# uci-rendering/psdr-cuda

Measured on AMD Instinct MI355X. Metric: Mpath-samples/s renderC+renderD, cbox 512x512 spp=64; grad rel-L2 vs ref, higher is better.
Workload: dtype f32; 1 GPU; cbox 512x512 spp=64/GPU PathTracer(max_depth=3): renderC + configure + renderD + enoki.forward w.r.t. diffuse albedo, through the psdr_cuda surface; triangles=12, global_spp=64, world_size=1, device=AMD Radeon Graphics, local_rank=0

## Files before the change

__graft_entry__.py:

```python
import os
import subprocess
import sys

ROOT = os.path.dirname(os.path.abspath(__file__))
PKG = os.path.join(ROOT, "psdr-cuda_amd")
for p in (PKG, os.path.join(ROOT, "oracle"), os.path.join(ROOT, "tests")):
    if p not in sys.path:
        sys.path.insert(0, p)

HIPCC_FLAGS = ["--offload-arch=gfx950", "-O3", "-std=c++17", "-fPIC", "-munsafe-fp-atomics",
               "-fno-hip-fp32-correctly-rounded-divide-sqrt", "-fgpu-flush-denormals-to-zero", "-fno-slp-vectorize",
               "-freciprocal-math", "-fapprox-func"]
VARIANTS = (0, 1, 2, 3, 4, 6, 8, 10)


def _stale(target, sources):
    return (not os.path.exists(target)) or any(os.path.getmtime(s) > os.path.getmtime(target) for s in sources)


def build():
    csrc = os.path.join(PKG, "csrc")
    srcs = [os.path.join(csrc, f) for f in os.listdir(csrc)] + [os.path.join(ROOT, "include", "psdr_hip.h")]
    lib = os.path.join(PKG, "lib", "libpsdr_hip.so")
    os.makedirs(os.path.dirname(lib), exist_ok=True)
    defect_job = None
    if _stale(lib, srcs):
        obj_dir = os.path.join(PKG, "lib", "obj")
        os.makedirs(obj_dir, exist_ok=True)
        jobs, objs, unit_cmds = [], [], {}
        for v in VARIANTS:
            o = os.path.join(obj_dir, "variant%d.o" % v)
            objs.append(o)
            unit_cmds[o] = ["hipcc"] + HIPCC_FLAGS + ["-DPSDR_VARIANT_FLAGS=%d" % v, "-c", os.path.join(csrc, "psdr_variant.hip"), "-o", o]
            jobs.append(subprocess.Popen(unit_cmds[o]))
            o = os.path.join(obj_dir, "path_sedge%d.o" % v)
            objs.append(o)
            unit_cmds[o] = ["hipcc"] + HIPCC_FLAGS + ["-DPSDR_VARIANT_FLAGS=%d" % v, "-c", os.path.join(csrc, "psdr_path_sedge.hip"), "-o", o]
            jobs.append(subprocess.Popen(unit_cmds[o]))
        o = os.path.join(obj_dir, "logd_lean.o")
        objs.append(o)
        unit_cmds[o] = ["hipcc"] + HIPCC_FLAGS + ["-c", os.path.join(csrc, "psdr_logd_lean.hip"), "-o", o]
        jobs.append(subprocess.Popen(unit_cmds[o]))
        o = os.path.join(obj_dir, "host.o")
        objs.append(o)
        unit_cmds[o] = ["hipcc"] + HIPCC_FLAGS + ["-c", os.path.join(csrc, "psdr_hip.hip"), "-o", o]
        jobs.append(subprocess.Popen(unit_cmds[o]))
        o = os.path.join(obj_dir, "tables.o")
        objs.append(o)
        unit_cmds[o] = ["hipcc"] + HIPCC_FLAGS + ["-c", os.path.join(csrc, "psdr_tables.hip"), "-o", o]
        jobs.append(subprocess.Popen(unit_cmds[o]))
        defect_job = _start_defect_object(csrc, obj_dir)
        if any(j.wait() != 0 for j in jobs):
            raise RuntimeError("hipcc failed")
        sys.path.insert(0, os.path.join(ROOT, "tools"))
        import check_spill_exec
        fallbacks = (["-mllvm", "-amdgpu-opt-exec-mask-pre-ra=0"], ["-mllvm", "-amdgpu-spill-sgpr-to-vgpr=0"])
        from concurrent.futures import ThreadPoolExecutor
        with ThreadPoolExecutor(max_workers=8) as pool:
            first = dict(zip(unit_cmds, pool.map(lambda o_: check_spill_exec.check_library(o_, verbose=True, min_code_objects=1), list(unit_cmds))))
        for o, cmd in list(unit_cmds.items()):
            hits = first[o]
            for extra in fallbacks:
                if not hits:
                    break
                print("build(): %s trips the spill guard -- rebuilding it with %s" % (os.path.basename(o), " ".join(extra)))
                subprocess.check_call(cmd[:1] + cmd[1:-4] + extra + cmd[-4:])
                hits = check_spill_exec.check_library(o, verbose=True, min_code_objects=1)
            if hits:
                raise RuntimeError("%s: %d kernel(s) spill in front of an exec restore with every fallback (tools/check_spill_exec.py)" % (os.path.basename(o), len(hits)))
        subprocess.check_call(["hipcc", "--offload-arch=gfx950", "-shared", "-fPIC"] + objs + ["-o", lib])
        if len(check_spill_exec.code_objects(lib)) < len(objs):
            raise RuntimeError("the linked library holds fewer gfx code objects than translation units: the spill guard cannot see all of it")
    subprocess.check_call(["make", "-C", os.path.join(ROOT, "oracle"), "-s"])
    hc_dir = os.path.join(ROOT, "tests", "hostcheck")
    hc = os.path.join(hc_dir, "libhostcheck.so")
    if _stale(hc, srcs + [os.path.join(hc_dir, "hostcheck.cpp")]):
        subprocess.check_call(["hipcc", "--offload-arch=gfx950", "-O2", "-std=c++17", "-fPIC", "-shared", "-pthread",
                               os.path.join(hc_dir, "hostcheck.cpp"), "-o", hc])
    hp = os.path.join(hc_dir, "libhostcheck_path_sedge.so")
    if _stale(hp, srcs + [os.path.join(hc_dir, "hostcheck_path_sedge.cpp")]):
        subprocess.check_call(["hipcc", "--offload-arch=gfx950", "-O2", "-std=c++17", "-fPIC", "-shared", "-pthread",
                               os.path.join(hc_dir, "hostcheck_path_sedge.cpp"), "-o", hp])
    po_dir = os.path.join(ROOT, "tests", "poison")
    po = os.path.join(po_dir, "libpoison.so")
    if _stale(po, [os.path.join(po_dir, "poison.hip")]):
        subprocess.check_call(["hipcc", "--offload-arch=gfx950", "-O1", "-fPIC", "-shared", os.path.join(po_dir, "poison.hip"), "-o", po])
    try:
        build_defect_lib(defect_job)
    except Exception as e:
        print("build(): tests/poison/libpsdr_hip_defect.so not built (%s) -- only tests/test_rough_rev_order_gpu.py uses it" % e)
    import psdr_cuda
    from psdr_cuda import _abi
    _abi.load_hip()
    import oracle
    oracle.load_oracle()


def _defect_object_cmd(csrc, obj_dir):
    return ["hipcc"] + HIPCC_FLAGS + ["-DPSDR_VARIANT_FLAGS=10", "-DPSDR_SINK_REG_PRIV_ROUGH=1", "-DPSDR_DPP_ALWAYS=1", "-c",
                                      os.path.join(csrc, "psdr_variant.hip"), "-o", os.path.join(obj_dir, "variant10_defect.o")]


def _start_defect_object(csrc, obj_dir):
    try:
        return subprocess.Popen(_defect_object_cmd(csrc, obj_dir), stdout=subprocess.DEVNULL, stderr=subprocess.DEVNULL)
    except Exception:
        return None


def build_defect_lib(object_job=None):
    csrc = os.path.join(PKG, "csrc")
    srcs = [os.path.join(csrc, f) for f in os.listdir(csrc)] + [os.path.join(ROOT, "include", "psdr_hip.h")]
    obj_dir = os.path.join(PKG, "lib", "obj")
    defect_lib = os.path.join(ROOT, "tests", "poison", "libpsdr_hip_defect.so")
    objs = [os.path.join(obj_dir, "%s%d.o" % (unit, v)) for v in VARIANTS for unit in ("variant", "path_sedge")] + [os.path.join(obj_dir, "logd_lean.o"), os.path.join(obj_dir, "host.o"), os.path.join(obj_dir, "tables.o")]
    if not all(os.path.exists(o) for o in objs):
        return None
    if object_job is not None and object_job.wait() != 0:
        object_job = None
    if _stale(defect_lib, srcs + objs):
        defect_obj = os.path.join(obj_dir, "variant10_defect.o")
        if object_job is None:
            subprocess.check_call(_defect_object_cmd(csrc, obj_dir))
        subprocess.check_call(["hipcc", "--offload-arch=gfx950", "-shared", "-fPIC"] + [defect_obj if o.endswith("variant10.o") else o for o in objs] + ["-o", defect_lib])
    return defect_lib


def smoke():
    import numpy as np
    import torch
    assert torch.cuda.is_available(), "smoke() needs a GPU"
    torch.cuda.set_device(0)
    import oracle
    from helpers import GpuScene, load_scene, rel_l2, tangents_wrt
    from psdr_cuda import _abi
    sc, P = load_scene("cbox", res=32, spp=8, sppe=4, sppse=4, translate=(0, (1.0, 0.0, 0.0)))
    tb = sc.tables(0)
    g = GpuScene(tb)
    o = _abi.make_opts(integrator=_abi.INTEGRATOR_PATH, max_depth=3, spp=8)
    img = g.render_c(o)
    ref = oracle.render(tb, o)
    assert np.isfinite(img).all() and rel_l2(img, ref) < 1e-4, rel_l2(img, ref)
    o = _abi.make_opts(spp=8, sppe=4, sppse=4)
    tan = tangents_wrt(tb, P)
    img, dimg = g.render_d_fwd(o, [tan])
    rimg, rd = oracle.render(tb, o, mode=1, tangents=tan)
    assert rel_l2(img, rimg) < 1e-4 and rel_l2(dimg[0], rd) < 1e-3, (rel_l2(img, rimg), rel_l2(dimg[0], rd))
    import psdr_cuda
    from psdr_cuda.fixtures import scene_path
    s2 = psdr_cuda.Scene()
    s2.load_file(scene_path("cbox"), False)
    s2.opts.width = s2.opts.height = 32
    s2.opts.spp, s2.opts.sppe, s2.opts.sppse, s2.opts.log_level = 4, 0, 0, 0
    s2.configure()
    out = psdr_cuda.DirectIntegrator(1, 1).renderC(s2).numpy()
    assert out.shape == (32 * 32, 3) and np.isfinite(out).all() and out.mean() > 0.05
    print("smoke OK: renderC rel-L2 vs oracle %.2e" % rel_l2(img, rimg))


if __name__ == "__main__":
    build()
    if len(sys.argv) > 1 and sys.argv[1] == "smoke":
        smoke()
    if len(sys.argv) > 1 and sys.argv[1] == "defect":
        print(build_defect_lib())
```

include/psdr_hip.h:

```cpp
#ifndef PSDR_HIP_H
#define PSDR_HIP_H

#include <stdint.h>

#ifdef __cplusplus
extern "C" {
#endif

#define PSDR_TRI_STRIDE   24
#define PSDR_TRIUV_STRIDE  8
#define PSDR_SEDGE_STRIDE 16
#define PSDR_PEDGE_STRIDE  8
#define PSDR_BSDF_STRIDE  16
#define PSDR_EMITTER_F_STRIDE 8
#define PSDR_EMITTER_I_STRIDE 4
#define PSDR_CAM_WORDS    64
#define PSDR_ENV_WORDS    32

#define PSDR_TRI_FACE_NORMALS 0x40000000

#define PSDR_BSDF_DIFFUSE        0
#define PSDR_BSDF_ROUGHCONDUCTOR 1
#define PSDR_SLOT_REFLECTANCE 0
#define PSDR_SLOT_ALPHA_U     1
// ... 102 lines not shown
    float *g_prim_edge;
    float *g_env_f;
} psdr_grads;

typedef struct psdr_scene_s *psdr_scene_t;

const char *psdr_last_error(void);
const char *psdr_version(void);
int psdr_abi_struct_sizes(int32_t out[4]);

int psdr_scene_create(psdr_scene_t *out);
int psdr_scene_destroy(psdr_scene_t h);
int psdr_scene_set_option(psdr_scene_t h, const char *name, double value);

int psdr_scene_set_tables(psdr_scene_t h, const psdr_scene_desc *desc);

int psdr_bvh_build(psdr_scene_t h, void *stream);
int psdr_bvh_stats(psdr_scene_t h, int32_t out[4]);
int psdr_scene_info(psdr_scene_t h, int32_t out[8]);

int psdr_trace(psdr_scene_t h, int32_t m,
               const float *ox, const float *oy, const float *oz,
               const float *dx, const float *dy, const float *dz,
               const float *tmax,
               int32_t *out_shape, int32_t *out_tri, float *out_u, float *out_v,
               void *stream);

int psdr_render_c(psdr_scene_t h, const psdr_render_opts *opts,
                  float *out_img, void *stream);

int psdr_render_d_fwd(psdr_scene_t h, const psdr_render_opts *opts,
                      int32_t K, const psdr_tangents *tangents,
                      float *out_img, float *out_dimg, void *stream);

int psdr_render_d_rev(psdr_scene_t h, const psdr_render_opts *opts,
                      const float *adj_img, float *out_img,
                      const psdr_grads *grads, void *stream);

int psdr_guide_build(psdr_scene_t h, const psdr_render_opts *opts,
                     const int32_t reso[4], int32_t nrounds,
                     float *out_mass, void *stream);

int psdr_cube_sample_reuse(int32_t ndim, const int32_t *reso, const float *cmf, const float *pmf, float sum,
                           int32_t n, int32_t m, float *samples, float *out_pdf, void *stream);
int psdr_sample_boundary_segment_direct(const psdr_scene_desc *desc, int32_t m, const float *sample3,
                                        const uint8_t *active, float *out_p0, float *out_edge_dir,
                                        float *out_edge2, float *out_p2, float *out_n, float *out_pdf,
                                        uint8_t *out_valid, int32_t *out_edge, float *out_s1, void *stream);

int psdr_geo_world_vertices_fwd(int32_t V, const float *v_raw, const int32_t *vmesh, const float *mats, float *v_world, void *stream);
int psdr_geo_world_vertices_rev(int32_t V, const float *v_raw, const int32_t *vmesh, const float *mats, const float *v_world, const float *a_world, float *a_raw,
                                void *stream);
int psdr_geo_world_vertices_jvp(int32_t V, const float *v_raw, const int32_t *vmesh, const float *mats, const float *v_world, const float *t_raw, const float *t_mats,
                                float *t_world, void *stream);
int psdr_geo_tri_rows_fwd(int32_t V, int32_t T, const float *v, const int32_t *faces, float *vsum, float *rows, int32_t row_stride, void *stream);
int psdr_geo_tri_rows_rev(int32_t V, int32_t T, const float *v, const int32_t *faces, const float *vsum, const float *a_rows, int32_t row_stride,
                          float *a_vsum , float *a_v, void *stream);
int psdr_geo_tri_rows_jvp(int32_t V, int32_t T, const float *v, const int32_t *faces, const float *vsum, const float *t_v, int32_t row_stride,
                          float *t_vsum , float *t_rows, void *stream);
int psdr_geo_sec_edges_fwd(int32_t E, const int32_t *edges, const float *v, const float *rows, int32_t row_stride, float *info, uint8_t *keep, void *stream);
int psdr_geo_sec_edges_rev(int32_t E, const int32_t *edges, const float *a_info, float *a_v, float *a_rows, int32_t row_stride, void *stream);
int psdr_geo_sec_edges_jvp(int32_t E, const int32_t *edges, const float *t_v, const float *t_rows, int32_t row_stride, float *t_info, void *stream);
int psdr_geo_prim_edges_fwd(int32_t E, const int32_t *edges, const uint8_t *face_normals, const float *v, const float *rows, int32_t row_stride,
                            const float *cam22, float *rows8, float *z4, uint8_t *keep, void *stream);
int psdr_geo_prim_edges_rev(int32_t E, const int32_t *edges, const float *v, const float *cam22, const float *a_rows8, float *a_v, float *a_w2s ,
                            void *stream);
int psdr_geo_prim_edges_jvp(int32_t E, const int32_t *edges, const float *v, const float *cam22, const float *t_v, const float *t_w2s , float *t_rows8,
                            void *stream);

int psdr_geo_compact_edges_fwd(int32_t E, const float *rows, int32_t S, const uint8_t *keep, int32_t w0, int32_t wn, const void *aux, int32_t aux_stride, int32_t A,
                               void *scratch, float *rows_out, void *aux_out, int32_t *pos, float *pmf, float *cmf, float *header, void *stream);
int psdr_geo_compact_edges_rev(int32_t E, int32_t S, const int32_t *pos, const float *a_rows_out, float *a_rows, void *stream);
int psdr_geo_compact_edges_jvp(int32_t E, int32_t S, const int32_t *pos, const float *t_rows, float *t_rows_out, void *stream);
int psdr_geo_emitter_tables(int32_t M, const float *rows, int32_t row_stride, const int32_t *face_offset, const int32_t *mesh_emitter, int32_t Ne, const int32_t *emitter_i,
                            const float *radiance, const float *env_weight, float *mesh_area, float *emitter_f, float *emitter_pmf, float *emitter_cmf, float *face_pmf,
                            float *face_cmf, void *stream);

int psdr_scene_rev_layout(psdr_scene_t h, int32_t out[16]);

int psdr_scene_seed_info(psdr_scene_t h, int64_t out[4]);

int psdr_scene_logd_info(psdr_scene_t h, int64_t out[4]);

int psdr_get_counters(psdr_scene_t h, uint64_t out[4]);

#ifdef __cplusplus
}
#endif
#endif
```

psdr-cuda_amd/csrc/psdr_device.h:

```cpp
#pragma once
#include "psdr_math.h"
#include "../../include/psdr_hip.h"

namespace psdr {

struct __attribute__((aligned(16))) BvhNode {
    float lo0[3], hi0[3];
    float lo1[3], hi1[3];
    int32_t c0, c1;
    int32_t pad[2];
};
static_assert(sizeof(BvhNode) == 64, "BvhNode must be 64 bytes");

struct __attribute__((aligned(16))) Bvh4Node {
    float org[3];
    uint32_t exps;
    uint32_t qlo[3], qhi[3];
    int32_t child[4];
    uint32_t pad[2];
};
static_assert(sizeof(Bvh4Node) == 64, "Bvh4Node must be 64 bytes");
constexpr int32_t kNoChild = 0x7ffffffe;

constexpr int kBvhStack = 40;
// ... 328 lines not shown
    if (sc.nodes4 != nullptr) walk_tree4<IGN>(sc, st, o, d, inv, root4, best, ig0, ig1);
    else walk_tree<IGN>(sc, st, o, d, inv, root2, best, ig0, ig1);
#else
    (void) root4; walk_tree<IGN>(sc, st, o, d, inv, root2, best, ig0, ig1);
#endif
}

#ifndef PSDR_PE_PAIR
#define PSDR_PE_PAIR 1
#endif
PSDR_HD void walk_tree_pair(const SceneView &sc, TraversalStack &st, const Vec3f &o, const Vec3f &dA, const Vec3f &invA, const Vec3f &dB, const Vec3f &invB, int32_t root,
                            Hit &bestA, Hit &bestB) {
    int sp = 0;
    int32_t cur = root;
    constexpr int32_t kDone = 0x7fffffff;
    while (cur != kDone) {
        while (cur >= 0 && cur != kDone) {
            BvhNode n;
#if defined(__HIP_DEVICE_COMPILE__)
            if (cur < sc.n_lnodes) n = *reinterpret_cast<const BvhNode *>(psdr_dyn_lds + sc.off_lnodes + cur * kLdsNodeStride);
            else
#endif
                n = sc.nodes[cur];
            float a0, a1, b0, b1;
            const bool hA0 = slab(n.lo0, n.hi0, o, invA, bestA.t, a0), hA1 = slab(n.lo1, n.hi1, o, invA, bestA.t, a1);
            const bool hB0 = slab(n.lo0, n.hi0, o, invB, bestB.t, b0), hB1 = slab(n.lo1, n.hi1, o, invB, bestB.t, b1);
            const bool h0 = hA0 || hB0, h1 = hA1 || hB1;
            if (h0 && h1) {
                const float t0 = fminf(hA0 ? a0 : INFINITY, hB0 ? b0 : INFINITY), t1 = fminf(hA1 ? a1 : INFINITY, hB1 ? b1 : INFINITY);
                const bool first0 = t0 <= t1;
                st.put(sp++, first0 ? n.c1 : n.c0);
                cur = first0 ? n.c0 : n.c1;
            } else if (h0 || h1) {
                cur = h0 ? n.c0 : n.c1;
            } else {
                cur = sp > 0 ? st.get(--sp) : kDone;
            }
        }
        if (cur == kDone) break;
        {
            const int enc = ~cur, first = enc >> 3, cnt = (enc & 7) + 1;
#if defined(__HIP_DEVICE_COMPILE__)
            if (first + cnt <= sc.n_lbtris) {
                const float4 *lt = reinterpret_cast<const float4 *>(psdr_dyn_lds + sc.off_lbtris) + first * 3;
                for (int i = 0; i < cnt; ++i) {
                    const float4 ta = lt[i * 3], tb = lt[i * 3 + 1], tc = lt[i * 3 + 2];
                    leaf_triangle_test<false>(ta, tb, tc, o, dA, bestA);
                    leaf_triangle_test<false>(ta, tb, tc, o, dB, bestB);
                }
            } else
#endif
            {
                const float4 *bt = sc.btris + (size_t) first * 3;
                for (int i = 0; i < cnt; ++i) {
                    const float4 ta = bt[i * 3], tb = bt[i * 3 + 1], tc = bt[i * 3 + 2];
                    leaf_triangle_test<false>(ta, tb, tc, o, dA, bestA);
                    leaf_triangle_test<false>(ta, tb, tc, o, dB, bestB);
                }
            }
            cur = sp > 0 ? st.get(--sp) : kDone;
        }
    }
}

PSDR_HD bool blas_box(const SceneView &sc, int k, const Vec3f &o, const Vec3f &inv, float tmax, float &t_entry) {
    const float lo[3] = {sc.blas_lo[k].x, sc.blas_lo[k].y, sc.blas_lo[k].z}, hi[3] = {sc.blas_hi[k].x, sc.blas_hi[k].y, sc.blas_hi[k].z};
    return slab(lo, hi, o, inv, tmax, t_entry);
}

PSDR_HD uint32_t wave_or_hd(uint32_t x) {
#if defined(__HIP_DEVICE_COMPILE__)
    unsigned long long todo = __ballot(1);
    uint32_t u = 0u;
    while (todo != 0ull) {
        const uint32_t f = (uint32_t) __builtin_amdgcn_readlane((int) x, __ffsll((long long) todo) - 1);
        u |= f;
        todo &= ~__ballot(x == f);
    }
    return u;
#else
    return x;
#endif
}
template <bool IGN = false, int FOREST = -1, bool MASKED = false>
PSDR_HD Hit closest_hit(const SceneView &sc, TraversalStack &st, const Vec3f &o, const Vec3f &d, float tmax, int ig0 = -1, int ig1 = -1, int pre_slot = 0, uint32_t rows = 0xffffffffu) {
    Hit best; best.tri = -1; best.u = best.v = -1.f;
    best.t = (tmax > 0.f && tmax < INFINITY) ? __int_as_float_hd(__float_as_int_hd(tmax) + 1) : tmax;
    const Vec3f inv{1.f / d.x, 1.f / d.y, 1.f / d.z};
    const bool forest = FOREST < 0 ? sc.n_blas > 0 : FOREST == 1;
    if (FOREST == 3 || FOREST == 2 || sc.n_tiny > 0 || forest) {
        int best_i = kNoPrim;
#if defined(__HIP_DEVICE_COMPILE__)
        typedef __attribute__((address_space(4))) const float4 kernarg_float4;
        const kernarg_float4 *prim_rows = (kernarg_float4 *) ((__attribute__((address_space(4))) const char *) __builtin_amdgcn_kernarg_segment_ptr() + offsetof(SceneView, tiny));
#else
        const float4 *prim_rows = sc.tiny;
#endif
        const int aa_cnt = sc.aa_cnt;
        if (aa_cnt != 0) {
            float4 ra[kAaSlots]; float hb[kAaSlots]; int pk[kAaSlots], id2[kAaSlots];
#pragma unroll
            for (int i = 0; i < kAaSlots; ++i) {
                ra[i] = prim_rows[i * 4];
                if (IGN) { const float4 r = prim_rows[i * 4 + 1]; hb[i] = r.x; pk[i] = __float_as_int_hd(r.y); id2[i] = __float_as_int_hd(r.w); }
                else {
#if defined(__HIP_DEVICE_COMPILE__)
                    const float2 r = *(__attribute__((address_space(4))) const float2 *) &prim_rows[i * 4 + 1];
#else
                    const float2 r{prim_rows[i * 4 + 1].x, prim_rows[i * 4 + 1].y};
#endif
                    hb[i] = r.x; pk[i] = __float_as_int_hd(r.y); id2[i] = 0;
                }
            }
            const int cx = aa_cnt & 255, cy = (aa_cnt >> 8) & 255, cz = aa_cnt >> 16;
#define PSDR_AA(AX, S) do { if (!MASKED || ((rows >> (S)) & 1u) != 0u) aa_prim_test<AX, IGN>(ra[S], hb[S], pk[S], id2[S], o, d, inv, best, best_i, ig0, ig1); } while (0)
            if (cx > 0) { PSDR_AA(0, 0); if (cx > 1) { PSDR_AA(0, 1); if (cx > 2) PSDR_AA(0, 2); } }
            if (cy > 0) { PSDR_AA(1, 3); if (cy > 1) { PSDR_AA(1, 4); if (cy > 2) PSDR_AA(1, 5); } }
            if (cz > 0) { PSDR_AA(2, 6); if (cz > 1) { PSDR_AA(2, 7); if (cz > 2) PSDR_AA(2, 8); } }
#undef PSDR_AA
        }
#pragma unroll PSDR_TINY_UNROLL
        for (int i = aa_cnt != 0 ? kAaSlots : 0; i < sc.n_tiny; ++i)
            if (!MASKED || ((rows >> i) & 1u) != 0u) tiny_prim_test<IGN>(prim_rows[i * 4], prim_rows[i * 4 + 1], prim_rows[i * 4 + 2], prim_rows[i * 4 + 3], i, o, d, best, best_i, ig0, ig1);
        resolve_tiny_hit(sc, best, best_i);
        if (FOREST == 3) {
            const Hit ph = st.pre[pre_slot];
            if (ph.tri >= 0 && ph.t < best.t) best = ph;
            return best;
        }
        if (FOREST == 2 || !forest) return best;
        if (sc.n_blas == 1) {
            float te;
            if (blas_box(sc, 0, o, inv, best.t, te)) walk<IGN>(sc, st, o, d, inv, __float_as_int_hd(sc.blas_lo[0].w), __float_as_int_hd(sc.blas_hi[0].w), best, ig0, ig1);
            return best;
        }
        uint32_t cand = (1u << sc.n_blas) - 1u;
        while (cand) {
            int32_t root = 0, root4 = 0; float near_t = INFINITY; uint32_t pick = 0;
            for (int k = 0; k < sc.n_blas; ++k) {
                if (!((cand >> k) & 1u)) continue;
                float te;
                if (!blas_box(sc, k, o, inv, best.t, te)) cand &= ~(1u << k);
                else if (te < near_t) { near_t = te; root = __float_as_int_hd(sc.blas_lo[k].w); root4 = __float_as_int_hd(sc.blas_hi[k].w); pick = 1u << k; }
            }
            if (!pick) break;
            cand &= ~pick;
            walk<IGN>(sc, st, o, d, inv, root, root4, best, ig0, ig1);
        }
        return best;
    }
    walk<IGN>(sc, st, o, d, inv, sc.root, sc.root4, best, ig0, ig1);
    return best;
}

template <int FLAGS> constexpr bool pair_walk_ok() { return PSDR_PE_PAIR != 0 && tree_mode<FLAGS>() == 1 && PSDR_WIDE_TREE == 0; }
PSDR_HD void closest_hit_pair(const SceneView &sc, TraversalStack &st, const Vec3f &o, const Vec3f &dA, const Vec3f &dB, Hit &hA, Hit &hB) {
#pragma unroll 1
    for (int r = 0; r < 2; ++r) {
        const Hit h = closest_hit<false, 2>(sc, st, o, r ? dB : dA, INFINITY);
        if (r) hB = h; else hA = h;
    }
    const Vec3f invA{1.f / dA.x, 1.f / dA.y, 1.f / dA.z}, invB{1.f / dB.x, 1.f / dB.y, 1.f / dB.z};
    for (int k = 0; k < sc.n_blas; ++k) {
        float te;
        const bool eA = blas_box(sc, k, o, invA, hA.t, te), eB = blas_box(sc, k, o, invB, hB.t, te);
        if (eA || eB) walk_tree_pair(sc, st, o, dA, invA, dB, invB, __float_as_int_hd(sc.blas_lo[k].w), hA, hB);
    }
}

template <class R> struct Loader;
template <> struct Loader<float> {
    template <int KK, int E> static PSDR_HD float f(const float *tab, const TangentView<KK, E> &, const float *const psdr_tangents::*, size_t i) { return tab[i]; }
};
template <int K> struct Loader<Dual<K>> {
    template <int E> static PSDR_HD Dual<K> f(const float *tab, const TangentView<K, E> &tv, const float *const psdr_tangents::*m, size_t i) {
        Dual<K> r; r.v = tab[i];
#pragma unroll
        for (int k = 0; k < K; ++k) { const float *p = tv.t[k].*m; r.d[k] = p ? p[i] : 0.f; }
        return r;
    }
};
template <class R, int FLAGS = kSceneRough> using TV = TangentView<ad_traits<R>::K, FLAGS>;
template <class R, class TVT> PSDR_HD R ldf(const float *tab, const TVT &tv, const float *const psdr_tangents::*m, size_t i) {
    return Loader<R>::f(tab, tv, m, i);
}
template <class R, class TVT> PSDR_HD Vec3<R> ld3(const float *tab, const TVT &tv, const float *const psdr_tangents::*m, size_t i) {
    return {ldf<R>(tab, tv, m, i), ldf<R>(tab, tv, m, i + 1), ldf<R>(tab, tv, m, i + 2)};
}
template <class M> PSDR_HD M to_m(float x) { return M(x); }
template <class M, int K> PSDR_HD M to_m(const Dual<K> &x) { return x; }
template <class M, class G> PSDR_HD Vec3<M> to_m3(const Vec3<G> &a) { return {to_m<M>(a.x), to_m<M>(a.y), to_m<M>(a.z)}; }

template <class R> struct TriRow { Vec3<R> p0, e1, e2, n0, n1, n2, fn; R area; };
template <class TVT> PSDR_HD TriRow<float> load_tri_f(const SceneView &sc, const TVT &, int id) {
    TriRow<float> t;
    float4 r[6];
#if defined(__HIP_DEVICE_COMPILE__)
    if (TVT::tiny || id < sc.n_ltri) {
        const float4 *q = reinterpret_cast<const float4 *>(psdr_dyn_lds + sc.off_ltri) + (size_t) id * 6;
#pragma unroll
        for (int i = 0; i < 6; ++i) r[i] = q[i];
    } else
#endif
    {
        const float4 *q = reinterpret_cast<const float4 *>(sc.d.tri_info) + (size_t) id * 6;
#pragma unroll
// ... 191 lines not shown
}

constexpr float kInvTwoPi = 0.15915494309189533577f;
template <class M, class G, class TVT> PSDR_HD Vec3<M> env_eval_direction(const SceneView &sc, const TVT &tv, const Vec3<G> &w) {
    const float *f = sc.d.env_f;
    constexpr auto m = &psdr_tangents::d_env_f;
    const Vec3<M> wm = to_m3<M>(w);
    auto row = [&](int r) {
        return ldf<M>(f, tv, m, PSDR_ENV_FROM_WORLD + r * 3) * wm.x + ldf<M>(f, tv, m, PSDR_ENV_FROM_WORLD + r * 3 + 1) * wm.y +
               ldf<M>(f, tv, m, PSDR_ENV_FROM_WORLD + r * 3 + 2) * wm.z;
    };
    const M vx = row(0), vy = row(1), vz = row(2);
    M u = atan2_(vx, -vz) * kInvTwoPi, v = safe_acos_(vy) * kInvPi;
    u = u - floorf(val(u)); v = v - floorf(val(v));
    M rgb[3];
    bitmap_eval<M, 3>(sc, tv, sc.d.env_tex, u, v, rgb, false);
    const M scale = ldf<M>(f, tv, m, PSDR_ENV_SCALE);
    return {rgb[0] * scale, rgb[1] * scale, rgb[2] * scale};
}
template <class M, class G, class TVT> PSDR_HD Vec3<M> Le(const SceneView &sc, const TVT &tv, const Its<G> &its, bool active) {
    const int e = active ? emitter_of(sc, tv, its) : -1;
    if (e < 0) return zero3<M>();
    if (TVT::has_env && e == sc.d.env_emitter) return env_eval_direction<M>(sc, tv, -its.sh.to_world(its.wi));
    if (!(val(its.wi.z) > 0.f)) return zero3<M>();
    return radiance<M>(sc, tv, e);
}


template <class R> struct GGX {
    R au, av;
    PSDR_HD R eval(const Vec3<R> &m) const {
        const R r = 1.f / (kPi * au * av * sqr(sqr(m.x / au) + sqr(m.y / av) + sqr(m.z)));
        return val(r) * val(m.z) > 1e-5f ? r : R(0.f);
    }
    PSDR_HD R smith_g1(const Vec3<R> &v, const Vec3<R> &m) const {
        const R xy = sqr(au * v.x) + sqr(av * v.y);
        R r = 2.f / (1.f + sqrt_(1.f + xy / sqr(v.z)));
        if (val(xy) == 0.f) r = R(1.f);
        if (val(dot(v, m)) * val(v.z) <= 0.f) r = R(0.f);
        return r;
    }
    PSDR_HD void visible11(const R &cos_i, float sx, float sy, R &ox, R &oy) const {
        float px, py;
        concentric_disk(sx, sy, px, py);
        const R s = 0.5f * (1.f + cos_i);
        const R y = sqrtf(fmaxf(1.f - px * px, 0.f)) * (1.f - s) + py * s;
        const R z = safe_sqrt(1.f - (px * px + y * y));
        const R sin_i = safe_sqrt(1.f - sqr(cos_i));
        const R nrm = 1.f / (sin_i * y + cos_i * z);
        ox = (cos_i * y - sin_i * z) * nrm; oy = px * nrm;
    }
    PSDR_HD Vec3<R> sample(const Vec3<R> &wi, float sx, float sy) const {
        const Vec3<R> wp = normalize(Vec3<R>(au * wi.x, av * wi.y, wi.z));
        const R st2 = wp.x * wp.x + wp.y * wp.y;
        R sin_phi(0.f), cos_phi(1.f);
        if (!(fabsf(val(st2)) <= 4.f * kEpsilon)) {
            const R inv = 1.f / sqrt_(st2);
            sin_phi = clamp_(wp.y * inv, -1.f, 1.f); cos_phi = clamp_(wp.x * inv, -1.f, 1.f);
        }
        R slx, sly;
        visible11(wp.z, sx, sy, slx, sly);
        const R s0 = (cos_phi * slx - sin_phi * sly) * au, s1 = (sin_phi * slx + cos_phi * sly) * av;
        return normalize(Vec3<R>(-s0, -s1, R(1.f)));
    }
};

template <class R> PSDR_HD R fresnel_conductor(const R &eta, const R &k, const R &cos_i) {
    const R c2 = sqr(cos_i), s2 = 1.f - c2, s4 = sqr(s2);
    const R t1 = sqr(eta) - sqr(k) - s2;
    const R a2pb2 = safe_sqrt(sqr(t1) + 4.f * sqr(k * eta));
    const R a = safe_sqrt(0.5f * (a2pb2 + t1));
    const R T1 = a2pb2 + c2, T2 = 2.f * cos_i * a;
    const R rs = (T1 - T2) / (T1 + T2);
    const R T3 = a2pb2 * c2 + s4, T4 = T2 * s2;
    return 0.5f * (rs + rs * (T3 - T4) / (T3 + T4));
}

template <class M> struct MatCache { M au, av; Vec3<M> eta, k, refl; };
template <class G, class M> struct Bsdf {
    const int32_t *rec;
    const MatCache<M> *mc = nullptr;
    PSDR_HD Bsdf(const SceneView &sc, int id) : rec(sc.d.bsdf_rec + (size_t) (id < 0 ? 0 : id) * PSDR_BSDF_STRIDE) {}
    template <class TVT> PSDR_HD Bsdf(const SceneView &sc, const TVT &, int id) : rec(Tab<TVT::flags>::bsdf_rec(sc, id)) {}
    template <class TVT> PSDR_HD MatCache<M> fetch(const SceneView &sc, const TVT &tv, const Its<G> &its) const {
        MatCache<M> c;
        c.refl = tex3(sc, tv, PSDR_SLOT_REFLECTANCE, its);
        if (is_diffuse(tv)) { c.au = c.av = M(0.f); c.eta = c.k = zero3<M>(); return c; }
        c.au = tex1(sc, tv, PSDR_SLOT_ALPHA_U, its); c.av = tex1(sc, tv, PSDR_SLOT_ALPHA_V, its);
        c.eta = tex3(sc, tv, PSDR_SLOT_ETA, its); c.k = tex3(sc, tv, PSDR_SLOT_K, its);
        return c;
    }
    PSDR_HD int type() const { return rec[0]; }
    template <class TVT> PSDR_HD bool is_diffuse(const TVT &) const { return !TVT::has_rough || rec[0] == PSDR_BSDF_DIFFUSE; }
    PSDR_HD const int32_t *slot(int s) const { return rec + 1 + 3 * s; }
    template <class TVT> PSDR_HD Vec3<M> tex3(const SceneView &sc, const TVT &tv, int s, const Its<G> &its) const {
        if (mc) return s == PSDR_SLOT_ETA ? mc->eta : (s == PSDR_SLOT_K ? mc->k : mc->refl);
        M o[3]; bitmap_eval<M, 3>(sc, tv, slot(s), its.uvx, its.uvy, o); return {o[0], o[1], o[2]};
    }
    template <class TVT> PSDR_HD M tex1(const SceneView &sc, const TVT &tv, int s, const Its<G> &its) const {
        if (mc) return s == PSDR_SLOT_ALPHA_U ? mc->au : mc->av;
        M o[1]; bitmap_eval<M, 1>(sc, tv, slot(s), its.uvx, its.uvy, o); return o[0];
    }
    template <class TVT> PSDR_HD Vec3<M> eval(const SceneView &sc, const TVT &tv, const Its<G> &its, const Vec3<G> &wo, bool active) const {
        if (!(active && val(its.wi.z) > 0.f && val(wo.z) > 0.f)) return zero3<M>();
        if (is_diffuse(tv)) return tex3(sc, tv, PSDR_SLOT_REFLECTANCE, its) * (wo.z * kInvPi);
        const GGX<M> g{tex1(sc, tv, PSDR_SLOT_ALPHA_U, its), tex1(sc, tv, PSDR_SLOT_ALPHA_V, its)};
        const Vec3<M> wi_m = to_m3<M>(its.wi), wo_m = to_m3<M>(wo);
        const Vec3<M> H = normalize(wo_m + wi_m);
        const M D = g.eval(H);
        if (val(D) == 0.f) return zero3<M>();
        const M res = D * (g.smith_g1(wi_m, H) * g.smith_g1(wo_m, H)) / (4.f * wi_m.z);
        const Vec3<M> eta = tex3(sc, tv, PSDR_SLOT_ETA, its), k = tex3(sc, tv, PSDR_SLOT_K, its);
        const M c = dot(wi_m, H);
        const Vec3<M> F{fresnel_conductor(eta.x, k.x, c), fresnel_conductor(eta.y, k.y, c), fresnel_conductor(eta.z, k.z, c)};
        return F * res * tex3(sc, tv, PSDR_SLOT_REFLECTANCE, its);
    }
    template <class TVT> PSDR_HD M pdf(const SceneView &sc, const TVT &tv, const Its<G> &its, const Vec3<G> &wo, bool active) const {
        if (is_diffuse(tv)) {
            const float ci = val(its.wi.z), co = val(wo.z);
            return M((active && ci > 0.f && co > 0.f) ? kInvPi * co : 0.f);
        }
        const Vec3<M> wi_m = to_m3<M>(its.wi);
        const Vec3<M> m = normalize(to_m3<M>(wo) + wi_m);
        const GGX<M> g{tex1(sc, tv, PSDR_SLOT_ALPHA_U, its), tex1(sc, tv, PSDR_SLOT_ALPHA_V, its)};
        return g.eval(m) * g.smith_g1(wi_m, m) / (4.f * wi_m.z);
    }
    template <class TVT> PSDR_HD bool sample(const SceneView &sc, const TVT &tv, const Its<G> &its, const float s[3], bool active, Vec3f &wo,
                                             M &pdf_) const {
        if (is_diffuse(tv)) {
            wo = cosine_hemisphere(s[1], s[2]);
            pdf_ = M(kInvPi * wo.z);
            return active && val(its.wi.z) > 0.f;
        }
        const GGX<M> g{tex1(sc, tv, PSDR_SLOT_ALPHA_U, its), tex1(sc, tv, PSDR_SLOT_ALPHA_V, its)};
        const Vec3<M> wi_m = to_m3<M>(its.wi);
        const Vec3<M> m = g.sample(wi_m, s[0], s[1]);
        const Vec3<M> wo_m = m * (2.f * dot(wi_m, m)) - wi_m;
        const Vec3<M> h = normalize(wo_m + wi_m);
        pdf_ = g.eval(h) * g.smith_g1(wi_m, h) / (4.f * wi_m.z);
        wo = val(wo_m);
        return active && val(its.wi.z) > 0.f && val(pdf_) != 0.f && wo.z > 0.f;
    }
};

template <class R> struct PosSample { Vec3<R> p, n; R J; float pdf; bool valid; int tri; };

template <int NDIM>
PSDR_HD float cube_sample_reuse(const float *__restrict__ cmf, const float *__restrict__ pmf, float sum, int n, int r0, int r1, int r2, float s[NDIM]) {
    static_assert(NDIM == 2 || NDIM == 3, "cube_sample_reuse: 2 or 3 dimensions");
    float p;
    const int idx = sample_reuse(cmf, pmf, sum, n, s[NDIM - 1], p);
    if constexpr (NDIM == 2) {
        const int c0 = idx / r1, c1 = idx - c0 * r1;
        s[0] = (s[0] + (float) c0) * (1.f / (float) r0);
        s[1] = (s[1] + (float) c1) * (1.f / (float) r1);
    } else {
        const int c0 = idx / (r1 * r2), rem = idx - c0 * r1 * r2, c1 = rem / r2, c2 = rem - c1 * r2;
        s[0] = (s[0] + (float) c0) * (1.f / (float) r0);
        s[1] = (s[1] + (float) c1) * (1.f / (float) r1);
        s[2] = (s[2] + (float) c2) * (1.f / (float) r2);
    }
    return p * (float) n;
}

PSDR_HD float env_cells_sample_reuse(const SceneView &sc, float &u0, float &u1) {
    const int r0 = sc.d.env_reso[0], r1 = sc.d.env_reso[1];
// ... 696 lines not shown
```

psdr-cuda_amd/csrc/psdr_hip.hip:

```cpp
#define PSDR_WIDE_TREE 2
#include "psdr_host.h"
#include "psdr_bvh_build.h"

#include <cstdlib>
#include <cstring>
#include <rocprim/rocprim.hpp>

namespace {
__global__ __launch_bounds__(kBlock) void k_trace(LaunchCtx cx, int m, const float *__restrict__ ox, const float *__restrict__ oy,
                                                  const float *__restrict__ oz, const float *__restrict__ dx,
                                                  const float *__restrict__ dy, const float *__restrict__ dz,
                                                  const float *__restrict__ tmax, int32_t *__restrict__ out_shape,
                                                  int32_t *__restrict__ out_tri, float *__restrict__ out_u, float *__restrict__ out_v) {
    TraversalStack st; setup_lds(cx, st);
    const SceneView &sc = cx.sc;
    for (int i = blockIdx.x * kBlock + threadIdx.x; i < m; i += gridDim.x * kBlock) {
        const Hit h = closest_hit<false, -1>(sc, st, Vec3f{ox[i], oy[i], oz[i]}, Vec3f{dx[i], dy[i], dz[i]}, tmax[i]);
        out_tri[i] = h.tri;
        out_shape[i] = h.tri >= 0 ? (sc.d.tri_mesh[h.tri] & ~PSDR_TRI_FACE_NORMALS) : -1;
        out_u[i] = h.u; out_v[i] = h.v;
    }
}


// ... 393 lines not shown
        if (hipMallocAsync(&nb, need, s) != hipSuccess) { (void) hipGetLastError(); nb = nullptr; }
    }
    if (*buf) HIP_TRY(hipFreeAsync(*buf, s));
    *buf = nullptr; *have = 0;
    if (nb == nullptr) {
        if (hipMallocAsync(&nb, need, s) != hipSuccess) {
            (void) hipGetLastError();
            return fail(std::string("psdr: could not allocate ") + std::to_string(need >> 20) + " MB of device memory for the " + what);
        }
    }
    *buf = nb; *have = need;
    return 0;
}

int launch_blocks(const psdr_scene_s *h, long long n, int per_cu) {
    const int forced = h->opt.blocks_per_cu;
    const long long need = (n + kBlock - 1) / kBlock;
    const long long cap = (long long) h->num_cus * (forced ? forced : per_cu);
    return (int) std::max(1LL, std::min(need, cap));
}

constexpr int kLdsBudget = 40 * 1024;
static bool tiny_only(const psdr_scene_s *h) { return h->n_tiny > 0 && h->n_blas == 0; }
static int emitter_faces(const psdr_scene_s *h) {
    int n = 0;
    for (int e = 0; e < h->desc.num_emitters && (size_t) (e + 1) * PSDR_EMITTER_I_STRIDE <= h->emitter_i.size(); ++e)
        n = std::max(n, h->emitter_i[(size_t) e * PSDR_EMITTER_I_STRIDE + 3] + h->emitter_i[(size_t) e * PSDR_EMITTER_I_STRIDE + 2]);
    return n;
}
constexpr int kLdsTexels = 256, kLdsTexelTangents = 3;
static bool small_tables_fit(const psdr_scene_s *h) {
    const psdr_scene_desc &d = h->desc;
    return d.env_emitter < 0 && d.num_meshes <= 64 && d.num_bsdfs <= 32 && d.num_emitters >= 0 && d.num_emitters <= 8 &&
           (d.num_emitters == 0 || (d.face_cmf && d.face_pmf)) && emitter_faces(h) <= 64;
}
static bool tiny_tables_ok(const psdr_scene_s *h) {
    return h->opt.tiny_variants != 0 && tiny_only(h) && small_tables_fit(h);
}
static bool forest_tables(const psdr_scene_s *h) { return PSDR_FOREST_LDS_TABLES && h->n_blas > 0; }
static bool use_wide_tree(const psdr_scene_s *h, bool forest) {
    if (h->opt.wide == 0) return false;
    return forest && h->has_rough && h->desc.env_emitter < 0;
}

static int stack_entries_of(const psdr_scene_s *h) { return tiny_only(h) ? 0 : (h->wide ? h->stack_need4 + 1 : std::min(kBvhStack, h->bvh_depth + 2)); }
static int staged_nodes_of(const psdr_scene_s *h) { return h->wide ? h->num_nodes4 : h->num_nodes; }
int plan_lds(const psdr_scene_s *h, LaunchCtx &cx, int reserved) {
    const int forced = h->opt.lds_budget;
    const bool lean = !h->has_rough && h->desc.env_emitter < 0;
    const int budget = forced ? forced : (lean ? 28 * 1024 : kLdsBudget);
    const int stack_bytes = stack_entries_of(h) * kBlock * 4;
    int room = std::max(0, budget - reserved - stack_bytes);
    if (tiny_only(h)) room = std::max(room, staged_nodes_of(h) * kLdsNodeStride + h->num_btris * 48 + h->desc.num_tris * 96);
    SceneView &sc = cx.sc;
    int off = 0;
    sc.n_lnodes = std::min(staged_nodes_of(h), room / kLdsNodeStride); sc.off_lnodes = off; off += sc.n_lnodes * kLdsNodeStride; room -= sc.n_lnodes * kLdsNodeStride;
    sc.n_lbtris = (sc.n_lnodes == staged_nodes_of(h)) ? std::min(h->num_btris, room / 48) : 0;
    sc.off_lbtris = off; off += sc.n_lbtris * 48; room -= sc.n_lbtris * 48;
    sc.n_ltri = (sc.n_lbtris == h->num_btris) ? std::min(h->desc.num_tris, room / 96) : 0;
    sc.off_ltri = off; off += sc.n_ltri * 96;
    sc.off_lprim = off; off += h->n_tiny * kTinyHitWords * 4;
    sc.lt_trimesh = sc.lt_meshbsdf = sc.lt_meshemitter = sc.lt_bsdf = sc.lt_emf = sc.lt_emi = sc.lt_fcmf = sc.lt_fpmf = sc.lt_uv = sc.lt_tex = sc.lt_ecmf = sc.lt_epmf = -1;
    sc.lt_nfaces = 0; sc.lt_occ = -1; sc.occ = nullptr;
    const bool all_tables = tiny_tables_ok(h);
    if (all_tables || forest_tables(h)) {
        auto take = [&](int words) { const int o = off; off += (words * 4 + 15) / 16 * 16; return o; };
        const psdr_scene_desc &d = h->desc;
        sc.lt_nfaces = emitter_faces(h);
        if (all_tables) sc.lt_trimesh = take(d.num_tris);
        sc.lt_meshbsdf = take(d.num_meshes); sc.lt_meshemitter = take(d.num_meshes);
        sc.lt_bsdf = take(std::max(d.num_bsdfs, 1) * PSDR_BSDF_STRIDE);
        sc.lt_emf = take(d.num_emitters * PSDR_EMITTER_F_STRIDE); sc.lt_emi = take(d.num_emitters * PSDR_EMITTER_I_STRIDE);
        sc.lt_fcmf = take(sc.lt_nfaces); sc.lt_fpmf = take(sc.lt_nfaces);
        if (d.num_emitters > 1 && d.emitter_cmf && d.emitter_pmf) { sc.lt_ecmf = take(d.num_emitters); sc.lt_epmf = take(d.num_emitters); }
        if (all_tables && d.tri_uv) sc.lt_uv = take(d.num_tris * PSDR_TRIUV_STRIDE);
        if (d.num_texels > 0 && d.num_texels <= kLdsTexels) sc.lt_tex = take(d.num_texels * (1 + kLdsTexelTangents));
        if (all_tables && h->have_occ && h->d_occ != nullptr) { sc.occ = h->d_occ; sc.lt_occ = take(d.num_tris * d.num_tris); }
    }
    sc.lt_end = off;
    cx.off_stack = off;
    return off + stack_bytes;
}
int lds_bytes(const LaunchCtx &cx, const psdr_scene_s *h) { return cx.off_stack + stack_entries_of(h) * kBlock * 4; }

void fill_top(const psdr_scene_s *h, SceneView &sc) {
    sc.n_tiny = h->n_tiny; sc.aa_cnt = h->n_tiny > 0 ? h->aa_cnt : 0;
    sc.emit_rows = (h->n_tiny > 0 && h->opt.emitter_pretest != 0) ? h->emit_rows : 0u;
    std::memcpy(sc.tiny, h->tiny, sizeof(h->tiny));
    std::memcpy(sc.tiny_meta, h->tiny_meta, sizeof(h->tiny_meta));
    sc.n_blas = h->n_blas;
    std::memcpy(sc.blas_lo, h->blas_lo, sizeof(h->blas_lo));
    std::memcpy(sc.blas_hi, h->blas_hi, sizeof(h->blas_hi));
    for (int k = 0; k < h->n_blas; ++k) std::memcpy(&sc.blas_hi[k].w, &h->blas_root4[k], 4);
    sc.nodes4 = h->wide ? h->d_nodes4 : nullptr; sc.root4 = h->root4;
}

int make_ctx(psdr_scene_s *h, const psdr_render_opts *o, int sampler, LaunchCtx &cx) {
    if (!h->have_tables) return fail("Scene not loaded yet!");
    if (!h->have_bvh) return fail("Input scene must be configured!");
    if (o->integrator != PSDR_INTEGRATOR_FIELD && h->desc.num_emitters <= 0) return fail("No Emitter!");
    if (o->integrator == PSDR_INTEGRATOR_DIRECT && !(o->bsdf_samples >= 0 && o->light_samples >= 0 && o->bsdf_samples + o->light_samples > 0))
        return fail("DirectIntegrator: bsdf_samples + light_samples must be positive");
    cx.sc.d = h->desc; cx.sc.nodes = h->d_nodes; cx.sc.btris = h->d_btris; cx.sc.root = h->root;
    fill_top(h, cx.sc);
    plan_lds(h, cx);
    cx.sc.literal_forms = (o->flags & PSDR_FLAG_LITERAL_FORMS) ? 1 : 0;
    cx.lp = LiParams{o->integrator, o->bsdf_samples, o->light_samples, o->max_depth, o->hide_emitters, o->field};
    cx.jump = make_rng_jump(o->rng_offset[sampler]);
    return 0;
}

int check_path_sedges(const psdr_render_opts *o) {
    if (o->integrator == PSDR_INTEGRATOR_PATH && (o->flags & PSDR_FLAG_PATH_SEDGES) != 0 && o->sppse > 0 && o->max_depth > PSDR_PATH_SEDGES_MAX_DEPTH)
        return fail("PSDR_FLAG_PATH_SEDGES: PathTracer max_depth > 8 is not supported for the secondary-edge term");
    return 0;
}
int check_counts(const psdr_scene_s *h, const psdr_render_opts *o) {
    const long long WH = (long long) h->desc.width * h->desc.height;
    if (WH <= 0) return fail("Invalid film resolution");
    if (WH * std::max(o->spp, 1) > 0x7fffffffLL) return fail("Too many samples (width*height*spp > INT_MAX)");
    if (o->spp_begin < 0 || o->spp_end > o->spp || o->spp_begin > o->spp_end) return fail("Invalid spp shard range");
    if (o->sppe_begin < 0 || o->sppe_end > o->sppe || o->sppe_begin > o->sppe_end) return fail("Invalid sppe shard range");
    if (o->sppse_begin < 0 || o->sppse_end > o->sppse || o->sppse_begin > o->sppse_end) return fail("Invalid sppse shard range");
    return 0;
}

bool open_scene(const psdr_scene_s *h) { return !(h->n_blas > 0 || (h->n_tiny > 0 && h->n_blas == 0)); }
bool use_wavefront(const psdr_scene_s *h, const psdr_render_opts *o) {
    if (o->integrator != PSDR_INTEGRATOR_PATH || o->max_depth > 250) return false;
    if (h->desc.num_tris >= (1 << 29)) return false;
    if (o->flags & PSDR_FLAG_FUSED) return false;
    if (o->flags & PSDR_FLAG_WAVEFRONT) return true;
    if (o->max_depth < 2) return false;
    if (open_scene(h)) return true;
    const long long n = (long long) h->desc.width * h->desc.height * (o->spp_end - o->spp_begin);
    if (traced_wavefront(h)) return n >= (1ll << 16);
    return h->n_blas > 0 && h->wf_binned && n >= (1ll << 25);
}

SinkLayout make_sink_layout(const psdr_scene_s *h, const psdr_grads *g) {
    SinkLayout L{};
    int off = 0;
    L.cam_off = off; off += 16;
    if (g->g_env_f && h->desc.env_emitter >= 0) { L.env_off = off; L.env_n = PSDR_ENV_WORDS; off += PSDR_ENV_WORDS; }
    const int nt = h->desc.num_texels, nr = h->desc.num_emitters * 3;
    if (g->g_texels && nt > 0 && nt <= 2048) { L.tex_off = off; L.tex_n = nt; off += nt; }
    if (g->g_emitter_rad && nr > 0 && nr <= 256) { L.rad_off = off; L.rad_n = nr; off += nr; }
    if (g->g_tri_info && h->hot_rows > 0) {
        const int rows = std::min(h->hot_rows, (kSinkCacheWords - off) / PSDR_TRI_STRIDE);
        if (rows > 0) { L.hot_off = off; L.hot_rows = rows; L.hot_map = h->d_hot_map; L.hot_tris = h->d_hot_tris; off += rows * PSDR_TRI_STRIDE; }
    }
    L.total = off;
    L.stride = off | 1;
    L.rep = 1;
    const int max_rep = h->opt.sink_rep;
    while (L.rep * 2 <= max_rep && L.rep * 2 * L.stride <= kSinkCacheWords) L.rep *= 2;
    const bool priv_on = h->opt.sink_private != 0;
    L.priv_tri[0] = L.priv_tri[1] = -1; L.priv_slot[0] = L.priv_slot[1] = 0; L.priv_emitter = -1;
    if (priv_on && L.hot_rows > 0 && h->desc.num_emitters > 0 && h->desc.env_emitter != 0) {
        const int32_t *ei = h->emitter_i.data();
        const int n = std::min(std::min(ei[2], 2), L.hot_rows);
        for (int r = 0; r < n; ++r) { L.priv_tri[r] = ei[1] + r; L.priv_slot[r] = h->hot_identity ? ei[1] + r : r; }
        L.priv_rows = n;
        if (n > 0) { L.priv_off = (L.rep * L.stride + 3) / 4 * 4; if (L.rad_n) L.priv_emitter = 0; }
    }
    return L;
// ... 272 lines not shown
    if (tiny_tables_ok(h)) fl |= kSceneTiny;
    switch (fl) {
        case 0: return variant_ops_0();
        case 1: return variant_ops_1();
        case 2: return variant_ops_2();
        case 3: return variant_ops_3();
        case 4: return variant_ops_4();
        case 8: return variant_ops_8();
        case 10: return variant_ops_10();
        default: return variant_ops_6();
    }
}
const PathSedgeOps *path_sedge_of(const psdr_scene_s *h) {
    int fl = (h->desc.env_emitter >= 0 ? kSceneEnv : 0) | (h->has_rough ? kSceneRough : 0) | (h->n_blas > 0 ? kSceneForest : 0);
    if (tiny_tables_ok(h)) fl |= kSceneTiny;
    switch (fl) {
        case 0: return path_sedge_ops_0();
        case 1: return path_sedge_ops_1();
        case 2: return path_sedge_ops_2();
        case 3: return path_sedge_ops_3();
        case 4: return path_sedge_ops_4();
        case 8: return path_sedge_ops_8();
        case 10: return path_sedge_ops_10();
        default: return path_sedge_ops_6();
    }
}
}
using namespace psdr_host;

extern "C" {

const char *psdr_last_error(void) { return g_err.c_str(); }
const char *psdr_version(void) { return "psdr-hip 0.1 gfx950"; }
int psdr_abi_struct_sizes(int32_t out[4]) {
    out[0] = (int32_t) sizeof(psdr_scene_desc); out[1] = (int32_t) sizeof(psdr_render_opts);
    out[2] = (int32_t) sizeof(psdr_tangents); out[3] = (int32_t) sizeof(psdr_grads);
    return 0;
}

int psdr_scene_create(psdr_scene_t *out) {
    if (!out) return fail("psdr_scene_create: null output");
    psdr_scene_s *h = new psdr_scene_s();
    hipError_t e = hipMalloc(&h->d_counters, sizeof(unsigned long long) * kRayCounters * kRayCounterStride);
    if (e != hipSuccess) { delete h; return fail(std::string("hipMalloc: ") + hipGetErrorString(e)); }
    int dev = 0; hipDeviceProp_t prop;
    if (hipGetDevice(&dev) == hipSuccess && hipGetDeviceProperties(&prop, dev) == hipSuccess) {
        h->num_cus = prop.multiProcessorCount;
        h->lds_limit = (int) std::min<size_t>(prop.sharedMemPerBlock, 160 * 1024);
    }
    *out = h;
    return 0;
}

int psdr_scene_set_option(psdr_scene_t h, const char *name, double value) {
    if (!h || !name) return fail("psdr_scene_set_option: null argument");
    const std::string n(name);
    const int iv = (int) value;
    if (n == "bvh_refit") h->refit_enabled = iv != 0;
    else if (n == "forest_min_inline") { h->forest_min_inline = iv; h->have_bvh = false; }
    else if (n == "scratch_plain") g_scratch_plain = iv;
    else if (n == "own_pixels") h->opt.own_pixels = iv;
    else if (n == "emitter_pretest") h->opt.emitter_pretest = iv;
    else if (n == "occ_rows") { h->opt.occ_rows = iv; h->have_bvh = false; }
    else if (n == "aa_prims") { h->aa_enabled = iv != 0; h->have_bvh = false; }
    else if (n == "tiny_scene") h->tiny_enabled = iv != 0;
    else if (n == "two_level") h->two_level_enabled = iv != 0;
    else if (n == "wf_binned") h->wf_binned = iv != 0;
    else if (n == "wf_traced") h->traced_enabled = iv != 0;
    else if (n == "bvh_build") h->bvh_device_mode = iv;
    else if (n == "sort_edges") h->sort_edges = iv != 0;
    else if (n == "blocks_per_cu") h->opt.blocks_per_cu = iv;
    else if (n == "camera_blocks") h->opt.camera_blocks = iv;
    else if (n == "tiny_variants") h->opt.tiny_variants = iv;
    else if (n == "wide") h->opt.wide = iv;
    else if (n == "lds_budget") h->opt.lds_budget = iv;
    else if (n == "sink_rep") h->opt.sink_rep = std::max(1, std::min(16, iv));
    else if (n == "sink_private") h->opt.sink_private = iv;
    else if (n == "rev_split") h->opt.rev_split = iv;
    else if (n == "tangent_live") h->opt.tangent_live = iv;
    else if (n == "wf_geo") h->opt.wf_geo = iv;
    else if (n == "logd") h->opt.logd = iv;
    else if (n == "seed_cache") h->opt.seed_cache = iv;
    else if (n == "logd_park") h->opt.logd_park = iv;
    else if (n == "seed_cache_log2") h->opt.seed_cache_log2 = std::max(0, std::min(40, iv));
    else if (n == "keep_records") h->opt.keep_records = iv;
    else if (n == "rev_sorted") h->opt.rev_sorted = iv;
    else if (n == "sedge_split") h->opt.sedge_split = iv;
    else if (n == "pt_sedge") h->opt.pt_sedge = iv & 3;
    else if (n == "pt_sedge_walk") h->opt.pt_sedge_walk = iv;
    else if (n == "probe") h->opt.probe = iv;
    else if (n == "trace_wg2") h->opt.trace_wg2 = iv;
    else if (n == "chunk_log2") h->opt.chunk_log2 = std::max(0, std::min(30, iv));
    else if (n == "bvh_maxleaf") h->opt.bvh_maxleaf = std::max(1, std::min(8, iv));
    else if (n == "bvh_tcost") h->opt.bvh_tcost = (float) value;
    else return fail("psdr_scene_set_option: unknown option '" + n + "'");
    h->kept.valid = false;
    if (n == "tiny_scene" || n == "two_level" || n == "bvh_build" || n == "wide" || n == "bvh_maxleaf" || n == "bvh_tcost" || n == "tiny_variants") h->have_bvh = false;
    return 0;
}

int psdr_scene_destroy(psdr_scene_t h) {
    if (!h) return 0;
    if (h->d_nodes) (void) hipFree(h->d_nodes);
    if (h->d_btris) (void) hipFree(h->d_btris);
    if (h->d_counters) (void) hipFree(h->d_counters);
    if (h->d_refit_area) (void) hipFree(h->d_refit_area);
    if (h->d_sort) (void) hipFree(h->d_sort);
    if (h->d_ws) (void) hipFree(h->d_ws);
    if (h->d_live) (void) hipFree(h->d_live);
    if (h->d_logd_bad) (void) hipFree(h->d_logd_bad);
    if (h->d_seed) (void) hipFree(h->d_seed);
    if (h->seed_event) (void) hipEventDestroy(h->seed_event);
    if (h->d_hot_map) (void) hipFree(h->d_hot_map);
    if (h->d_hot_tris) (void) hipFree(h->d_hot_tris);
    if (h->d_occ) (void) hipFree(h->d_occ);
    if (h->d_top) (void) hipFree(h->d_top);
    if (h->d_inline_ids) (void) hipFree(h->d_inline_ids);
    if (h->d_lbvh) (void) hipFree(h->d_lbvh);
    if (h->d_nodes4) (void) hipFree(h->d_nodes4);
    if (h->d_topo4) (void) hipFree(h->d_topo4);
    if (h->d_rev) (void) hipFree(h->d_rev);
    if (h->d_se_list) (void) hipFree(h->d_se_list);
    if (h->d_rev_deep) (void) hipFree(h->d_rev_deep);
    if (h->d_pe_rep) (void) hipFree(h->d_pe_rep);
    if (h->d_trace_ovf) (void) hipFree(h->d_trace_ovf);
    if (h->d_probe) (void) hipFree(h->d_probe);
    delete h;
    return 0;
}

int psdr_scene_set_tables(psdr_scene_t h, const psdr_scene_desc *desc) {
    if (!h || !desc) return fail("psdr_scene_set_tables: null argument");
    psdr_scene_desc d = *desc;
    if (d.num_tris <= 0 || !d.tri_info || !d.tri_mesh) return fail("Missing meshes!");
    if (!d.cam) return fail("Missing sensor!");
    if (reinterpret_cast<uintptr_t>(d.tri_info) & 15) return fail("psdr_scene_set_tables: tri_info must be 16-byte aligned");
    if (d.width <= 0 || d.height <= 0) return fail("Invalid film resolution");
    if (d.num_meshes <= 0 || !d.mesh_bsdf || !d.mesh_emitter) return fail("psdr_scene_set_tables: mesh_bsdf / mesh_emitter missing");
    if (d.num_bsdfs > 0 && (!d.bsdf_rec || !d.texels)) return fail("psdr_scene_set_tables: bsdf_rec / texels missing");
    if (d.num_emitters > 0 && (!d.emitter_f || !d.emitter_i)) return fail("psdr_scene_set_tables: emitter tables missing");
    if (d.num_emitters > 1 && (!d.emitter_cmf || !d.emitter_pmf)) return fail("psdr_scene_set_tables: emitter distribution missing");
    if (d.num_sec_edges > 0 && (!d.sec_edge || !d.sec_cmf || !d.sec_pmf)) return fail("psdr_scene_set_tables: secondary-edge tables missing");
    if (d.num_prim_edges > 0 && (!d.prim_edge || !d.prim_cmf || !d.prim_pmf)) return fail("psdr_scene_set_tables: primary-edge tables missing");
    if (d.num_prim_edges <= 0) d.prim_edge_z = nullptr;
    if (d.num_guide_cells > 0 && (!d.guide_cmf || !d.guide_pmf)) return fail("psdr_scene_set_tables: guiding tables missing");
    if (!d.env_f) d.env_emitter = -1;
    if (d.env_emitter >= 0) {
        if (d.env_emitter >= d.num_emitters || !d.env_cmf || !d.env_pmf || d.env_reso[0] <= 0 || d.env_reso[1] <= 0 || d.env_tex[1] < 2 ||
            d.env_tex[2] < 2)
            return fail("psdr_scene_set_tables: inconsistent environment-map record");
    }
    if (h->have_tables && (d.tri_info != h->desc.tri_info || d.num_tris != h->desc.num_tris)) h->have_bvh = false;
    if (h->have_tables && (d.emitter_i != h->desc.emitter_i || d.num_emitters != h->desc.num_emitters)) h->have_bvh = false;
    if (!h->have_tables || std::memcmp(&h->desc, &d, sizeof(d)) != 0) { ++h->tables_gen; h->kept.valid = false; }
    h->desc = d;
    h->has_rough = d.material_mask == 0 || (d.material_mask & (1u << PSDR_BSDF_ROUGHCONDUCTOR)) != 0;
    h->have_tables = true;
    return 0;
}

static hipError_t copy_on_stream(void *dst, const void *src, size_t bytes, hipMemcpyKind kind, hipStream_t s) {
    if (hipError_t e = hipMemcpyAsync(dst, src, bytes, kind, s)) return e;
    return hipStreamSynchronize(s);
}
static void update_emit_rows(psdr_scene_s *h) {
    std::vector<char> is_em((size_t) std::max(h->desc.num_tris, 0), 0);
// ... 291 lines not shown
    if (n <= 0 || n > 0x7fffffffLL) return fail("psdr_guide_build: invalid resolution");
    HIP_TRY(hipMemsetAsync(out_mass, 0, sizeof(float) * cells, s));
    return variant_of(h)->guide(h, cx, reso, nrounds, n, out_mass, s);
}

int psdr_cube_sample_reuse(int32_t ndim, const int32_t *reso, const float *cmf, const float *pmf, float sum, int32_t n, int32_t m, float *samples,
                           float *out_pdf, void *stream) {
    if (!reso || !cmf || !pmf || !samples || !out_pdf) return fail("psdr_cube_sample_reuse: null argument");
    if (ndim != 2 && ndim != 3) return fail("psdr_cube_sample_reuse: ndim must be 2 or 3");
    long long cells = 1;
    for (int d = 0; d < ndim; ++d) {
        if (reso[d] <= 0) return fail("psdr_cube_sample_reuse: invalid resolution");
        cells *= reso[d];
    }
    if (cells != (long long) n) return fail("psdr_cube_sample_reuse: n must be the product of the resolution");
    if (m < 0) return fail("psdr_cube_sample_reuse: negative sample count");
    if (m == 0) return 0;
    const dim3 grid((unsigned) ((m + kBlock - 1) / kBlock));
    hipStream_t s = (hipStream_t) stream;
    if (ndim == 2)
        hipLaunchKernelGGL(k_cube_sample_reuse<2>, grid, dim3(kBlock), 0, s, m, cmf, pmf, sum, n, reso[0], reso[1], 1, samples, out_pdf);
    else
        hipLaunchKernelGGL(k_cube_sample_reuse<3>, grid, dim3(kBlock), 0, s, m, cmf, pmf, sum, n, reso[0], reso[1], reso[2], samples, out_pdf);
    HIP_TRY(hipGetLastError());
    return 0;
}

int psdr_sample_boundary_segment_direct(const psdr_scene_desc *desc, int32_t m, const float *sample3, const uint8_t *active, float *out_p0,
                                        float *out_edge_dir, float *out_edge2, float *out_p2, float *out_n, float *out_pdf, uint8_t *out_valid,
                                        int32_t *out_edge, float *out_s1, void *stream) {
    if (!desc || !sample3 || !out_p0 || !out_edge_dir || !out_edge2 || !out_p2 || !out_n || !out_pdf || !out_valid || !out_edge || !out_s1)
        return fail("psdr_sample_boundary_segment_direct: null argument");
    const psdr_scene_desc &d = *desc;
    if (d.num_sec_edges <= 0 || !d.sec_edge || !d.sec_cmf || !d.sec_pmf) return fail("Scene has no secondary edges");
    if (d.num_emitters <= 0 || !d.emitter_f || !d.emitter_i) return fail("No Emitter!");
    if (d.num_emitters > 1 && (!d.emitter_cmf || !d.emitter_pmf)) return fail("psdr_sample_boundary_segment_direct: emitter distribution missing");
    const bool env = d.env_f != nullptr && d.env_emitter >= 0;
    if (env && (d.env_emitter >= d.num_emitters || !d.env_cmf || !d.env_pmf || d.env_reso[0] <= 0 || d.env_reso[1] <= 0))
        return fail("psdr_sample_boundary_segment_direct: inconsistent environment-map record");
    if (d.num_emitters > (env ? 1 : 0) && (d.num_tris <= 0 || !d.tri_info || !d.face_cmf || !d.face_pmf))
        return fail("psdr_sample_boundary_segment_direct: area-light tables missing");
    if (m < 0) return fail("psdr_sample_boundary_segment_direct: negative sample count");
    if (m == 0) return 0;
    SceneView sc{};
    sc.d = d;
    if (!env) sc.d.env_emitter = -1;
    const dim3 grid((unsigned) ((m + kBlock - 1) / kBlock));
    hipStream_t s = (hipStream_t) stream;
    if (env)
        hipLaunchKernelGGL(k_boundary_segment_direct<kSceneEnv>, grid, dim3(kBlock), 0, s, sc, m, sample3, active, out_p0, out_edge_dir, out_edge2, out_p2, out_n,
                           out_pdf, out_valid, out_edge, out_s1);
    else
        hipLaunchKernelGGL(k_boundary_segment_direct<0>, grid, dim3(kBlock), 0, s, sc, m, sample3, active, out_p0, out_edge_dir, out_edge2, out_p2, out_n,
                           out_pdf, out_valid, out_edge, out_s1);
    HIP_TRY(hipGetLastError());
    return 0;
}

int psdr_bvh_stats(psdr_scene_t h, int32_t out[4]) {
    if (!h || !out) return fail("psdr_bvh_stats: null argument");
    out[0] = h->num_builds; out[1] = h->num_refits; out[2] = h->num_nodes; out[3] = h->bvh_depth;
    return 0;
}

int psdr_scene_info(psdr_scene_t h, int32_t out[8]) {
    if (!h || !out) return fail("psdr_scene_info: null argument");
    const int n_slab = (h->aa_cnt & 255) + ((h->aa_cnt >> 8) & 255) + (h->aa_cnt >> 16);
    out[0] = h->n_tiny - (h->aa_cnt != 0 ? kAaSlots - n_slab : 0); out[1] = h->n_blas; out[2] = h->n_inline; out[3] = h->num_btris; out[4] = h->lbvh ? 1 : 0;
    out[5] = n_slab; out[6] = h->have_occ ? 1 : 0; out[7] = h->have_occ ? h->occ_max_rows : 0;
    return 0;
}

int psdr_scene_rev_layout(psdr_scene_t h, int32_t out[16]) {
    if (!h || !out) return fail("psdr_scene_rev_layout: null argument");
    std::copy(std::begin(h->rev_layout), std::end(h->rev_layout), out);
    return 0;
}

int psdr_scene_logd_info(psdr_scene_t h, int64_t out[4]) {
    if (!h || !out) return fail("psdr_scene_logd_info: null argument");
    out[0] = h->logd_launches; out[1] = h->logd_lean_launches; out[2] = h->logd_lean_seeded; out[3] = (int64_t) h->logd_lean_lds + h->logd_lean_park;
    return 0;
}
int psdr_scene_seed_info(psdr_scene_t h, int64_t out[4]) {
    if (!h || !out) return fail("psdr_scene_seed_info: null argument");
    out[0] = h->seed_valid ? h->seed_key[0] * h->seed_key[3] : 0; out[1] = (int64_t) (h->seed_cap * sizeof(ulonglong2)); out[2] = h->seed_fills; out[3] = h->seed_launches;
    return 0;
}

int psdr_get_counters(psdr_scene_t h, uint64_t out[4]) {
    if (!h || !out) return fail("psdr_get_counters: null argument");
    unsigned long long all[kRayCounters * kRayCounterStride], c[1] = {0};
    HIP_TRY(hipMemcpyAsync(all, h->d_counters, sizeof(all), hipMemcpyDeviceToHost, h->last_stream));
    HIP_TRY(hipStreamSynchronize(h->last_stream));
    for (int i = 0; i < kRayCounters; ++i) c[0] += all[i * kRayCounterStride];
#ifdef PSDR_STAGE_CLOCKS
    {
        unsigned long long ph[12] = {0};
        for (int i = 0; i < kRayCounters; ++i) for (int k = 0; k < 12; ++k) ph[k] += all[i * kRayCounterStride + 1 + k];
        std::fprintf(stderr, "stage clocks:");
        for (int k = 0; k < 12; ++k) std::fprintf(stderr, " %llu", ph[k]);
        std::fprintf(stderr, "\n");
    }
#endif
    out[0] = c[0]; out[1] = h->slots[0]; out[2] = h->slots[1]; out[3] = h->slots[2];
    return 0;
}

}
```

psdr-cuda_amd/csrc/psdr_host.h:

```cpp
#pragma once
#include "psdr_device.h"
#include "psdr_reverse.h"

#include <algorithm>
#include <type_traits>
#include <cmath>
#include <cstdio>
#include <cstdlib>
#include <cstring>
#include <string>
#include <vector>

using namespace psdr;

struct LaunchCtx {
    SceneView sc;
    LiParams lp;
    RngJump jump;
    int32_t off_stack;
    int32_t off_pathrec;
    int32_t off_sink;
    int32_t off_park;
};

static_assert(offsetof(LaunchCtx, sc) == 0, "closest_hit reads SceneView::tiny through the kernel-argument segment pointer: LaunchCtx (SceneView first) must be the first kernel argument");

__device__ __forceinline__ void setup_lds(const LaunchCtx &cx, TraversalStack &st) {
#if defined(__HIP_DEVICE_COMPILE__)
    const SceneView &sc = cx.sc;
    float4 *dst = reinterpret_cast<float4 *>(psdr_dyn_lds);
    const float4 *src = sc.nodes4 != nullptr ? reinterpret_cast<const float4 *>(sc.nodes4) : reinterpret_cast<const float4 *>(sc.nodes);
    for (int i = threadIdx.x; i < sc.n_lnodes * 4; i += kBlock) dst[sc.off_lnodes / 16 + (i >> 2) * (kLdsNodeStride / 16) + (i & 3)] = src[i];
    for (int i = threadIdx.x; i < sc.n_lbtris * 3; i += kBlock) dst[sc.off_lbtris / 16 + i] = sc.btris[i];
    src = reinterpret_cast<const float4 *>(sc.d.tri_info);
    for (int i = threadIdx.x; i < sc.n_ltri * 6; i += kBlock) dst[sc.off_ltri / 16 + i] = src[i];
    {
        float *m = reinterpret_cast<float *>(psdr_dyn_lds + sc.off_lprim);
#pragma unroll 1
        for (int i = 0; i < sc.n_tiny; ++i) {
            int32_t tri; float k[6];
            const int w = threadIdx.x & 7;
            const float4 Sm = sc.tiny[i * 4 + 2];
            const float S[4] = {Sm.x, Sm.y, Sm.z, Sm.w};
            tiny_hit_row(sc.tiny_meta + i * 4, (threadIdx.x >> 3) & 1, tri, k, (sc.aa_cnt != 0 && i < kAaSlots) ? S : nullptr);
            const float val = w == 0 ? __int_as_float(tri) : (w == 1 ? k[0] : w == 2 ? k[1] : w == 3 ? k[2] : w == 4 ? k[3] : w == 5 ? k[4] : w == 6 ? k[5] : 0.f);
            if (threadIdx.x < kTinyHitWords) m[i * kTinyHitWords + threadIdx.x] = val;
        }
    }
    if (sc.lt_meshbsdf >= 0) {
        auto stage = [&](int off, const void *table, int words) {
            if (off < 0 || table == nullptr) return;
            const uint32_t *g = static_cast<const uint32_t *>(table);
            uint32_t *l = reinterpret_cast<uint32_t *>(psdr_dyn_lds + off);
#pragma unroll 1
            for (int i = threadIdx.x; i < words; i += kBlock) l[i] = g[i];
        };
        stage(sc.lt_trimesh, sc.d.tri_mesh, sc.d.num_tris);
        stage(sc.lt_meshbsdf, sc.d.mesh_bsdf, sc.d.num_meshes);
        stage(sc.lt_meshemitter, sc.d.mesh_emitter, sc.d.num_meshes);
        stage(sc.lt_bsdf, sc.d.bsdf_rec, sc.d.num_bsdfs * PSDR_BSDF_STRIDE);
        stage(sc.lt_emf, sc.d.emitter_f, sc.d.num_emitters * PSDR_EMITTER_F_STRIDE);
        stage(sc.lt_emi, sc.d.emitter_i, sc.d.num_emitters * PSDR_EMITTER_I_STRIDE);
        stage(sc.lt_ecmf, sc.d.emitter_cmf, sc.d.num_emitters);
        stage(sc.lt_epmf, sc.d.emitter_pmf, sc.d.num_emitters);
        stage(sc.lt_fcmf, sc.d.face_cmf, sc.lt_nfaces);
        stage(sc.lt_fpmf, sc.d.face_pmf, sc.lt_nfaces);
        stage(sc.lt_uv, sc.d.tri_uv, sc.d.num_tris * PSDR_TRIUV_STRIDE);
        stage(sc.lt_tex, sc.d.texels, sc.d.num_texels);
        stage(sc.lt_occ, sc.occ, sc.d.num_tris * sc.d.num_tris);
    }
    st.base = reinterpret_cast<int32_t *>(psdr_dyn_lds + cx.off_stack) + threadIdx.x;
    __syncthreads();
#else
    (void) cx; (void) st;
#endif
}
template <class TVT> __device__ __forceinline__ void setup_lds(const LaunchCtx &cx, TraversalStack &st, const TVT &tv) {
    setup_lds(cx, st);
#if defined(__HIP_DEVICE_COMPILE__)
    if constexpr (Tab<TVT::flags>::lds_small && TVT::k > 0) {
        constexpr int K = TVT::k;
        static_assert(K <= 3, "plan_lds reserves three tangent texel pools");
        if (cx.sc.lt_tex >= 0) {
            float *l = reinterpret_cast<float *>(psdr_dyn_lds + cx.sc.lt_tex);
            const int nt = cx.sc.d.num_texels;
            for (int k = 0; k < K; ++k) {
                const float *g = tv.t[k].d_texels;
                for (int i = threadIdx.x; i < nt; i += kBlock) l[(k + 1) * nt + i] = g ? g[i] : 0.f;
            }
            __syncthreads();
        }
    }
#endif
}

constexpr int kSinkCacheWords = 6144;
struct SinkLayout {
    int tex_off, tex_n;
    int rad_off, rad_n;
    int cam_off;
    int env_off, env_n;
    int hot_off, hot_rows;
    const int32_t *hot_map, *hot_tris;
    int total;
    int rep, stride;
    int priv_off, priv_rows;
    int priv_tri[2], priv_slot[2], priv_emitter;
    int priv_regs;
    int pend_off, pend_rows;
};
constexpr int kPendWords = 10;
constexpr int kPrivRowWords = 13;
constexpr int kPrivWords = 2 * kPrivRowWords + 3;

struct psdr_scene_options {
    int blocks_per_cu = 0;
    int camera_blocks = 0;
    int tiny_variants = 1;
    int wide = -1;
    int lds_budget = 0;
    int sink_rep = 4;
    int sink_private = 1;
    int rev_split = -1;
    int tangent_live = 1;
    int wf_geo = 1;
    int own_pixels = 1;
    int emitter_pretest = 1;
    int occ_rows = 1;
    int logd = 1;
    int keep_records = 1;
    int rev_sorted = 1;
    int pt_sedge = 3;
    int pt_sedge_walk = 1;
    int sedge_split = -1;
    int chunk_log2 = 0;
    int probe = 1;
    int trace_wg2 = -1;
    int seed_cache = 1;
    int seed_cache_log2 = 25;
    int logd_park = 1;
    int bvh_maxleaf = 4;
    float bvh_tcost = 2.0f;
};

struct psdr_scene_s {
    psdr_scene_options opt;
    psdr_scene_desc desc{};
    bool have_tables = false;
    bool has_rough = true;
    int num_cus = 256;
    int lds_limit = 64 * 1024;

    BvhNode *d_nodes = nullptr;
    float4 *d_btris = nullptr;
    size_t cap_nodes = 0, cap_btris = 0;
    int32_t root = 0;
    bool have_bvh = false;
    int bvh_depth = 0, num_nodes = 0, num_btris = 0;
    Bvh4Node *d_nodes4 = nullptr;
    int32_t *d_topo4 = nullptr;
    size_t cap_nodes4 = 0;
    int num_nodes4 = 0, stack_need4 = 0;
    bool wide = false;
    int32_t *d_trace_ovf = nullptr;
    size_t trace_ovf_bytes = 0;
    bool traced_enabled = true;
    int32_t root4 = 0, blas_root4[kMaxBlas] = {};
    bool refit_enabled = true;
    int tree_tris = -1, refits_since_build = 0, num_builds = 0, num_refits = 0;
    std::vector<int> level_start;
    float bvh_pad = 0.f, built_area = 0.f;
    float *d_refit_area = nullptr;

    int bvh_device_mode = -1;
    bool lbvh = false;
    int lbvh_leaves = 0;
    void *d_lbvh = nullptr;
    size_t lbvh_bytes = 0;

    bool tiny_enabled = true, aa_enabled = true;
    int n_tiny = 0, aa_cnt = 0;
    float4 tiny[kTinyRows * 4] = {};
    int32_t tiny_meta[kTinyRows * 4] = {};
    bool two_level_enabled = true, refit_ok = true, wf_binned = true;
    int n_blas = 0, n_inline = 0;
    float4 blas_lo[kMaxBlas] = {}, blas_hi[kMaxBlas] = {};
    float4 *d_top = nullptr;
    int32_t *d_inline_ids = nullptr;

    unsigned long long *d_counters = nullptr;
    hipStream_t last_stream = nullptr;
    hipStream_t refit_stream = nullptr;
    uint64_t slots[3] = {0, 0, 0};
    int last_path_depth = 0;
    int32_t rev_layout[16] = {};

    std::vector<int32_t> emitter_i;
    int32_t *d_hot_map = nullptr, *d_hot_tris = nullptr;
    uint32_t *d_occ = nullptr; size_t occ_cap = 0; bool have_occ = false; int occ_max_rows = 0;
    int hot_rows = 0;
    bool hot_identity = false;
    size_t hot_cap = 0;

    bool sort_edges = true;
    void *d_sort = nullptr;
    size_t sort_bytes = 0;

    void *d_pe_rep = nullptr;
    size_t pe_rep_bytes = 0;

    void *d_rev_deep = nullptr;
    size_t rev_deep_bytes = 0;

    void *d_se_list = nullptr;
    size_t se_list_bytes = 0;

    void *d_rev = nullptr;
    size_t rev_bytes = 0;
    void *d_logd_bad = nullptr; size_t logd_bad_bytes = 0;
    struct KeptRecords { bool valid = false; psdr_render_opts o{}; uint64_t gen = 0; long long n = 0; int kind = 0; } kept;
    uint64_t tables_gen = 0;

    void *d_seed = nullptr;
    size_t seed_cap = 0;
    long long seed_key[4] = {0, 0, 0, 0};
    bool seed_valid = false;
    hipStream_t seed_stream = nullptr;
    hipEvent_t seed_event = nullptr;
    long long seed_fills = 0, seed_launches = 0;
    long long logd_launches = 0, logd_lean_launches = 0, logd_lean_seeded = 0;
    int logd_lean_lds = 0, logd_lean_park = 0;
    void *d_ws = nullptr;
    size_t ws_bytes = 0;
    void *d_live = nullptr;
    size_t live_bytes = 0;
    void *d_probe = nullptr;
    size_t probe_bytes = 0;
    uint32_t emit_rows = 0;
    int forest_min_inline = 0;
};

constexpr int kRayCounters = 64, kRayCounterStride = 16;
constexpr int kWfSub = 64, kWfCountStride = 32;

namespace psdr_host {
int fail(const std::string &m);
int scratch_reserve(void **buf, size_t *have, size_t need, hipStream_t s, const char *what);
long long fit_chunk(long long chunk, size_t bytes_per_slot, size_t fixed_bytes, size_t have);
inline int workspace_reserve(psdr_scene_s *h, size_t need, hipStream_t s) { return scratch_reserve(&h->d_ws, &h->ws_bytes, need, s, "wavefront workspace (path-state streams + trace requests)"); }
int launch_blocks(const psdr_scene_s *h, long long n, int per_cu = 16);
int plan_lds(const psdr_scene_s *h, LaunchCtx &cx, int reserved = 0);
int lds_bytes(const LaunchCtx &cx, const psdr_scene_s *h);
void fill_top(const psdr_scene_s *h, SceneView &sc);
constexpr int kMaxInlineTris = 2 * kTinyTris;
int make_ctx(psdr_scene_s *h, const psdr_render_opts *o, int sampler, LaunchCtx &cx);
bool use_wavefront(const psdr_scene_s *h, const psdr_render_opts *o);
bool traced_wavefront(const psdr_scene_s *h);
int launch_wf_trace(psdr_scene_s *h, const float4 *req, const int32_t *count, long long sub_cap, float4 *hit, hipStream_t s, bool ign = false);
struct ProbeBuffers { float4 *hit; uint32_t *mask; float4 *req; int32_t *count; long long sub_cap; };
int probe_buffers(psdr_scene_s *h, long long slots, int rays_per_slot, ProbeBuffers &pb, hipStream_t s, int per_cu = 16);
SinkLayout make_sink_layout(const psdr_scene_s *h, const psdr_grads *g);
inline int sink_bytes_base(const SinkLayout &L) { return (L.priv_rows > 0 && !L.priv_regs) ? (L.priv_off + kPrivWords * kBlock) * 4 : (L.rep * L.stride * 4 + 15) / 16 * 16; }
inline int sink_bytes(const SinkLayout &L) { return L.pend_rows > 0 ? (L.pend_off + L.pend_rows * kPendWords * kBlock) * 4 : sink_bytes_base(L); }
inline void sink_reserve_pending(SinkLayout &L, int rows) { L.pend_rows = 0; L.pend_off = (sink_bytes_base(L) / 4 + 3) / 4 * 4; L.pend_rows = rows; }
int check_counts(const psdr_scene_s *h, const psdr_render_opts *o);
int begin_call(psdr_scene_s *h, hipStream_t s);
int primary_edge_order(psdr_scene_s *h, const LaunchCtx &cx, long long i0, long long n, const uint32_t **order, hipStream_t s);
constexpr int kMaxRefits = 64;
constexpr float kRefitAreaGrowth = 1.3f;

struct VariantOps {
    int (*render_c)(psdr_scene_s *h, const psdr_render_opts *o, float *img, hipStream_t s);
    int (*render_fwd)(psdr_scene_s *h, const psdr_render_opts *o, int K, const psdr_tangents *tangents, float *img, float *dimg, hipStream_t s);
    int (*render_rev)(psdr_scene_s *h, const psdr_render_opts *o, const float *adj_img, float *out_img, const psdr_grads *grads, hipStream_t s);
    int (*guide)(psdr_scene_s *h, LaunchCtx &cx, const int32_t reso[4], int nrounds, long long n, float *out_mass, hipStream_t s);
};
struct PathSedgeOps {
    int (*fwd)(psdr_scene_s *h, const psdr_render_opts *o, int K, const psdr_tangents *tangents, float *dimg, hipStream_t s);
    int (*rev)(psdr_scene_s *h, const psdr_render_opts *o, const float *adj_img, const psdr_grads *grads, hipStream_t s);
};
const PathSedgeOps *path_sedge_ops_0();
const PathSedgeOps *path_sedge_ops_1();
const PathSedgeOps *path_sedge_ops_2();
const PathSedgeOps *path_sedge_ops_3();
const PathSedgeOps *path_sedge_ops_4();
const PathSedgeOps *path_sedge_ops_6();
const PathSedgeOps *path_sedge_ops_8();
const PathSedgeOps *path_sedge_ops_10();
int logd_lean_launch_8(psdr_scene_s *h, const psdr_render_opts *o, const LaunchCtx &cx, const psdr::TangentView<1, psdr::kSceneTiny> &tv, float *img, float *dimg, hipStream_t s, bool *ran);
const VariantOps *variant_ops_0();
const VariantOps *variant_ops_1();
const VariantOps *variant_ops_2();
const VariantOps *variant_ops_3();
const VariantOps *variant_ops_4();
const VariantOps *variant_ops_6();
const VariantOps *variant_ops_8();
const VariantOps *variant_ops_10();
}

#define HIP_TRY(expr)                                                                              \
    do { hipError_t e_ = (expr); if (e_ != hipSuccess) return psdr_host::fail(std::string(#expr) + ": " + hipGetErrorString(e_)); } while (0)
```

psdr-cuda_amd/csrc/psdr_kernels.h:

```cpp
#pragma once
#include "psdr_host.h"

namespace {
using namespace psdr_host;

__device__ __forceinline__ float wave_shfl_down(float v, int off) { return __shfl_down(v, off, 64); }

template <int CTRL, int ROW_MASK> __device__ __forceinline__ float dpp_add(float v) {
    return v + __int_as_float(__builtin_amdgcn_update_dpp(0, __float_as_int(v), CTRL, ROW_MASK, 0xf, true));
}
__device__ __forceinline__ float wave_total(float v) {
    v = dpp_add<0x111, 0xf>(v); v = dpp_add<0x112, 0xf>(v); v = dpp_add<0x114, 0xf>(v); v = dpp_add<0x118, 0xf>(v);
    v = dpp_add<0x142, 0xa>(v); v = dpp_add<0x143, 0xc>(v);
    return __int_as_float(__builtin_amdgcn_readlane(__float_as_int(v), 63));
}
#ifndef PSDR_DPP_ALWAYS
#define PSDR_DPP_ALWAYS 0
#endif
template <int N, bool DPP = (N <= 6 || PSDR_DPP_ALWAYS)> __device__ __forceinline__ bool wave_segmented_sum(int key, float (&v)[N]) {
    const int lane = threadIdx.x & 63;
    if (DPP && __ballot(key != __builtin_amdgcn_readfirstlane(key)) == 0ull) {
#pragma unroll
        for (int i = 0; i < N; ++i) v[i] = wave_total(v[i]);
        return lane == 0;
// ... 1479 lines not shown
}
inline int big_launch_per_cu(const psdr_scene_s *h, long long n) { return (int) std::max(16LL, std::min(40LL, n / ((long long) kBlock * h->num_cus * 8))); }
inline long long launch_chunk(const psdr_scene_s *h, int log2_default) { return 1ll << (h->opt.chunk_log2 > 0 ? h->opt.chunk_log2 : log2_default); }
inline bool probe_direct(const psdr_scene_s *h, const psdr_render_opts *o, long long n) {
    return traced_wavefront(h) && h->opt.probe != 0 && o->bsdf_samples == 1 && o->light_samples == 1 && !(o->flags & PSDR_FLAG_FUSED) && n >= (1ll << 16);
}
inline const ulonglong2 *seed_table(psdr_scene_s *h, const psdr_render_opts *o, long long WH, int nsp, long long n, hipStream_t s) {
    if (h->opt.seed_cache == 0 || n <= 0 || n > (1ll << std::max(0, std::min(40, h->opt.seed_cache_log2)))) return nullptr;
    const long long key[4] = {WH, (long long) o->spp, (long long) o->spp_begin, (long long) nsp};
    if (h->d_seed != nullptr && h->seed_valid && std::equal(key, key + 4, h->seed_key)) {
        if (s != h->seed_stream && h->seed_event != nullptr && hipStreamWaitEvent(s, h->seed_event, 0) != hipSuccess) { (void) hipGetLastError(); return nullptr; }
        return reinterpret_cast<const ulonglong2 *>(h->d_seed);
    }
    h->seed_valid = false;
    if ((size_t) n > h->seed_cap) {
        if (h->d_seed) { (void) hipFreeAsync(h->d_seed, s); h->d_seed = nullptr; h->seed_cap = 0; }
        void *nb = nullptr;
        if (hipMallocAsync(&nb, (size_t) n * sizeof(ulonglong2), s) != hipSuccess) { (void) hipGetLastError(); return nullptr; }
        h->d_seed = nb; h->seed_cap = (size_t) n;
    }
    if (h->seed_event == nullptr && hipEventCreateWithFlags(&h->seed_event, hipEventDisableTiming) != hipSuccess) { (void) hipGetLastError(); h->seed_event = nullptr; return nullptr; }
    hipLaunchKernelGGL(k_seed_fill, dim3((unsigned) ((n + kBlock - 1) / kBlock)), dim3(kBlock), 0, s, reinterpret_cast<ulonglong2 *>(h->d_seed), n, o->spp, o->spp_begin, SlotDiv(nsp));
    if (hipGetLastError() != hipSuccess || hipEventRecord(h->seed_event, s) != hipSuccess) { (void) hipGetLastError(); return nullptr; }
    std::copy(key, key + 4, h->seed_key);
    h->seed_valid = true; h->seed_stream = s; h->seed_fills++;
    return reinterpret_cast<const ulonglong2 *>(h->d_seed);
}
template <class G, class R, int FL> constexpr bool seeded_render_c() { return (FL & kSceneTiny) != 0 && (FL & kScenePre) == 0 && std::is_same<G, float>::value && std::is_same<R, float>::value; }
template <class G, class R, int FL>
int run_camera(psdr_scene_s *h, const psdr_render_opts *o, const TV<R, FL> &tv, float *img, float *dimg, hipStream_t s) {
    const long long WH = (long long) h->desc.width * h->desc.height;
    const int nsp = o->spp_end - o->spp_begin;
    if (o->spp <= 0 || nsp <= 0) return 0;
    LaunchCtx cx;
    if (int rc = make_ctx(h, o, 0, cx)) return rc;
    const long long n = WH * nsp;
    h->slots[0] += (uint64_t) n;
    const int own = (h->opt.own_pixels != 0 && nsp <= 64 && 64 % nsp == 0) ? 1 : 0;
    if constexpr ((FL & kSceneForest) != 0) {
        if (o->integrator == PSDR_INTEGRATOR_DIRECT && probe_direct(h, o, n)) {
            const TangentView<0, FL> tv0{};
            TV<R, FL | kScenePre> tvp;
            for (int k = 0; k < (ad_traits<R>::K > 0 ? ad_traits<R>::K : 1); ++k) tvp.t[k] = tv.t[k];
            tvp.live = tv.live;
            LaunchCtx cxp = cx;
            plan_lds(h, cxp, 1 << 30);
            cxp.sc.n_lnodes = cxp.sc.n_lbtris = cxp.sc.n_ltri = 0;
            const long long chunk = std::min<long long>(n, launch_chunk(h, 25));
            for (long long c0 = 0; c0 < n; c0 += chunk) {
                const long long nc = std::min(chunk, n - c0);
                ProbeBuffers pb;
                const int probe_per_cu = big_launch_per_cu(h, nc);
                if (int rc = probe_buffers(h, nc, 3, pb, s, probe_per_cu)) return rc;
                const TraceQueue tq{pb.req, pb.count, pb.sub_cap};
                const int blocks = (launch_blocks(h, nc, probe_per_cu) + kWfSub - 1) / kWfSub * kWfSub;
                hipLaunchKernelGGL(k_direct_probe<FL>, dim3(blocks), dim3(kBlock), lds_bytes(cx, h), s, cx, tv0, o->spp, o->spp_begin, SlotDiv(nsp), c0, nc, tq, pb.hit, pb.mask,
                                   make_rng_jump(o->rng_offset[0] + 2));
                HIP_TRY(hipGetLastError());
                if (int rc = launch_wf_trace(h, pb.req, pb.count, pb.sub_cap, pb.hit, s)) return rc;
                hipLaunchKernelGGL(HIP_KERNEL_NAME(k_camera<G, R, PSDR_INTEGRATOR_DIRECT, FL | kScenePre, false>), dim3(launch_blocks(h, nc, camera_blocks_per_cu(h, nc))), dim3(kBlock), cxp.off_stack, s,
                                   cxp, tvp, o->spp, o->spp_begin, SlotDiv(nsp), nc, 1.f / (float) o->spp, img, dimg, WH * 3, h->d_counters, c0, ProbeView{pb.hit, pb.mask}, own);
                HIP_TRY(hipGetLastError());
            }
            return 0;
        }
    }
    bool gated = false;
    if constexpr (logd_instance<G, R, PSDR_INTEGRATOR_PATH, FL>()) {
        constexpr int K = ad_traits<R>::K;
        bool texels_only = o->integrator == PSDR_INTEGRATOR_PATH && h->opt.logd != 0 && h->desc.num_texels > 0 && h->desc.texels != nullptr;
        for (int k = 0; k < K && texels_only; ++k) {
            const psdr_tangents &t = tv.t[k];
            texels_only = t.d_texels != nullptr && !t.d_tri_info && !t.d_emitter_rad && !t.d_cam_to_world && !t.d_sec_edge && !t.d_prim_edge && !t.d_env_f;
        }
        if (texels_only) {
            if (int rc = scratch_reserve(&h->d_logd_bad, &h->logd_bad_bytes, sizeof(int), s, "log-derivative gate")) return rc;
            int *bad = reinterpret_cast<int *>(h->d_logd_bad);
            HIP_TRY(hipMemsetAsync(bad, 0, sizeof(int), s));
            TangentView<K, 0> tvk;
            for (int k = 0; k < K; ++k) tvk.t[k] = tv.t[k];
            hipLaunchKernelGGL(k_logd_check<K>, dim3((unsigned) ((h->desc.num_texels + kBlock - 1) / kBlock)), dim3(kBlock), 0, s, h->desc.texels, tvk, h->desc.num_texels, h->d_counters, bad);
            hipLaunchKernelGGL(k_logd_gate, dim3(1), dim3(64), 0, s, h->d_counters, bad);
            bool lean = false;
            if constexpr (K == 1 && FL == kSceneTiny) { if (int rc = logd_lean_launch_8(h, o, cx, tv, img, dimg, s, &lean)) return rc; }
            if (!lean)
                hipLaunchKernelGGL(HIP_KERNEL_NAME(k_camera_logd<K, FL, ((FL & kSceneTiny) != 0)>), dim3(launch_blocks(h, n, camera_blocks_per_cu(h, n))), dim3(kBlock), lds_bytes(cx, h), s, cx, tv,
                                   o->spp, o->spp_begin, SlotDiv(nsp), n, 1.f / (float) o->spp, img, dimg, WH * 3, h->d_counters, own);
            HIP_TRY(hipGetLastError());
            h->logd_launches++;
            gated = true;
        }
    }
#define PSDR_LAUNCH_CAMERA_T(INTEG, NOTREE)                                                                                        \
    hipLaunchKernelGGL(HIP_KERNEL_NAME(k_camera<G, R, INTEG, FL, NOTREE>), dim3(launch_blocks(h, n, camera_blocks_per_cu(h, n))), dim3(kBlock), lds_bytes(cx, h), s, cx, tv, o->spp, \
                       o->spp_begin, nsp, n, 1.f / (float) o->spp, img, dimg, WH * 3, h->d_counters, 0ll, ProbeView{nullptr, nullptr}, own)
#define PSDR_LAUNCH_CAMERA(INTEG) PSDR_LAUNCH_CAMERA_T(INTEG, ((FL & kSceneTiny) != 0))
    if constexpr (seeded_render_c<G, R, FL>()) {
        if (o->integrator == PSDR_INTEGRATOR_PATH) {
            if (const ulonglong2 *seed = seed_table(h, o, WH, nsp, n, s)) {
                hipLaunchKernelGGL(HIP_KERNEL_NAME(k_camera_seeded<G, R, PSDR_INTEGRATOR_PATH, FL, true>), dim3(launch_blocks(h, n, camera_blocks_per_cu(h, n))), dim3(kBlock), lds_bytes(cx, h), s, cx, tv,
                                   o->spp, o->spp_begin, SlotDiv(nsp), n, 1.f / (float) o->spp, img, dimg, WH * 3, h->d_counters, own, seed);
                HIP_TRY(hipGetLastError());
                h->seed_launches++;
                return 0;
            }
        }
    }
    switch (o->integrator) {
        case PSDR_INTEGRATOR_DIRECT: PSDR_LAUNCH_CAMERA(PSDR_INTEGRATOR_DIRECT); break;
        case PSDR_INTEGRATOR_PATH: PSDR_LAUNCH_CAMERA(PSDR_INTEGRATOR_PATH); break;
        case PSDR_INTEGRATOR_FIELD: PSDR_LAUNCH_CAMERA(PSDR_INTEGRATOR_FIELD); break;
        default: return fail("Unknown integrator");
    }
#undef PSDR_LAUNCH_CAMERA
#undef PSDR_LAUNCH_CAMERA_T
    HIP_TRY(hipGetLastError());
    if (gated) HIP_TRY(hipMemsetAsync(h->d_counters + kLogdGateWord, 0, sizeof(unsigned long long), s));
    return 0;
}


constexpr int kWfMaxDepth = 256;
struct WfRecArgs { float *disk; long long stride, c0, nc; };
template <class M, int FL>
int run_camera_wavefront(psdr_scene_s *h, const psdr_render_opts *o, const TV<M, FL> &tv, float *img, float *dimg, hipStream_t s, const WfRecArgs *rec = nullptr) {
    constexpr int K = ad_traits<M>::K;
    const long long WH = (long long) h->desc.width * h->desc.height;
    const int nsp = o->spp_end - o->spp_begin;
    if (o->spp <= 0 || nsp <= 0) return 0;
    const long long n_all = WH * nsp;
    const long long n = rec ? rec->nc : n_all;
    bool traced = false;
    if constexpr ((FL & kSceneForest) != 0) traced = traced_wavefront(h);
    const bool binned = !traced && (FL & kSceneForest) != 0 && h->n_blas > 0 && h->wf_binned;
    const int depth = o->max_depth;
    const size_t words = 8 + 6 * (1 + K) + (traced ? 8 : 0);
    const long long cap = rec ? n : std::min(n, fit_chunk(binned ? launch_chunk(h, 24) : launch_chunk(h, traced ? 26 : 25), 2 * words * 4 * 5 / 4 + (traced ? 80 : 0), 64u << 20, h->ws_bytes));
    const auto wf_per_cu = [&](long long slots) { return traced ? big_launch_per_cu(h, slots) : 16; };
    const long long max_blocks = ((long long) launch_blocks(h, cap, wf_per_cu(cap)) + kWfSub - 1) / kWfSub * kWfSub;
    const long long binned_sub_cap = (((cap + kBlock - 1) / kBlock + kWfSub) / kWfGroups + 2) * kBlock;
    const long long cap_alloc = ((binned ? binned_sub_cap * kWfSub : cap + max_blocks * kBlock) + 63) / 64 * 64;
    const size_t cnt_ints = (size_t) (kWfMaxDepth + 1) * kWfStageInts + (traced ? (size_t) (kWfMaxDepth + 1) * kWfSub * kWfCountStride : 0);
    const size_t cnt_bytes = cnt_ints * sizeof(int32_t);
    const size_t req_bytes = traced ? (size_t) 2 * cap_alloc * 2 * sizeof(float4) : 0;
    const size_t need = 2 * words * 4 * (size_t) cap_alloc + cnt_bytes + req_bytes;
    if (int rc = workspace_reserve(h, need, s)) return rc;
    int32_t *cnt = reinterpret_cast<int32_t *>(h->d_ws);
    int32_t *req_cnt = cnt + (size_t) (kWfMaxDepth + 1) * kWfStageInts;
    PathStream st[2];
    for (int i = 0; i < 2; ++i) {
        float *b = reinterpret_cast<float *>(reinterpret_cast<char *>(h->d_ws) + cnt_bytes) + (size_t) i * words * cap_alloc;
        const long long c = cap_alloc;
        st[i].cap = c;
        st[i].pixel = reinterpret_cast<int32_t *>(b); st[i].slot = reinterpret_cast<uint32_t *>(b + c); st[i].tri = reinterpret_cast<int32_t *>(b + 2 * c);
        st[i].hu = b + 3 * c; st[i].hv = b + 4 * c; st[i].dir = b + 5 * c; st[i].beta = b + 8 * c; st[i].acc = b + (8 + 3 * (1 + K)) * c;
        st[i].hit = traced ? reinterpret_cast<float4 *>(b + (8 + 6 * (1 + K)) * c) : nullptr;
        st[i].prev_t = nullptr;
        st[i].binned = binned ? 1 : 0;
    }
    TraceQueue tq{};
    tq.req = traced ? reinterpret_cast<float4 *>(reinterpret_cast<char *>(h->d_ws) + cnt_bytes + 2 * words * 4 * (size_t) cap_alloc) : nullptr;
    if (!rec) h->slots[0] += (uint64_t) n;
    const float inv_spp = 1.f / (float) o->spp;
    const long long j_first = rec ? rec->c0 : 0;
    for (long long j0 = j_first; j0 < j_first + n; j0 += cap) {
        const long long cn = std::min(cap, j_first + n - j0);
        LaunchCtx cx;
        if (int rc = make_ctx(h, o, 0, cx)) return rc;
        HIP_TRY(hipMemsetAsync(cnt, 0, (size_t) (std::min(depth, kWfMaxDepth) + 1) * kWfStageInts * sizeof(int32_t), s));
        if (traced) HIP_TRY(hipMemsetAsync(req_cnt, 0, (size_t) (std::min(depth, kWfMaxDepth) + 1) * kWfSub * kWfCountStride * sizeof(int32_t), s));
        const int blocks = (launch_blocks(h, cn, wf_per_cu(cn)) + kWfSub - 1) / kWfSub * kWfSub;
        const long long trips = (cn + (long long) blocks * kBlock - 1) / ((long long) blocks * kBlock);
        st[0].sub_cap = st[1].sub_cap = binned ? binned_sub_cap : (blocks / kWfSub) * trips * kBlock;
        st[0].count = cnt;
        if constexpr ((FL & kSceneForest) != 0) {
            if (traced) {
                tq.sub_cap = 2 * st[0].sub_cap;
                tq.count = req_cnt;
                LaunchCtx cxp = cx;
                plan_lds(h, cxp, 1 << 30);
                cxp.sc.n_lnodes = cxp.sc.n_lbtris = cxp.sc.n_ltri = 0;
                const int dyn_p = cxp.off_stack;
// ... 546 lines not shown
```

psdr-cuda_amd/psdr_cuda/_abi.py:

```python
import ctypes as C
import os

_HERE = os.path.dirname(os.path.abspath(__file__))
PKG_ROOT = os.path.dirname(_HERE)
REPO_ROOT = os.path.dirname(PKG_ROOT)

TRI_STRIDE = 24
TRIUV_STRIDE = 8
SEDGE_STRIDE = 16
PEDGE_STRIDE = 8
BSDF_STRIDE = 16
EMITTER_F_STRIDE = 8
EMITTER_I_STRIDE = 4
CAM_WORDS = 64
ENV_WORDS = 32
TRI_FACE_NORMALS = 0x40000000

BSDF_DIFFUSE, BSDF_ROUGHCONDUCTOR = 0, 1
SLOT_REFLECTANCE, SLOT_ALPHA_U, SLOT_ALPHA_V, SLOT_ETA, SLOT_K = range(5)
CAM_SAMPLE_TO_CAMERA, CAM_TO_WORLD, CAM_WORLD_TO_SAMPLE, CAM_POS, CAM_DIR, CAM_INV_AREA = 0, 16, 32, 48, 51, 54
INTEGRATOR_DIRECT, INTEGRATOR_PATH, INTEGRATOR_FIELD = 0, 1, 2
FLAG_FUSED, FLAG_WAVEFRONT, FLAG_LITERAL_FORMS, FLAG_KEEP_RECORDS, FLAG_PATH_SEDGES = 1, 2, 4, 8, 16
MAX_PATH_SEDGE_DEPTH = 8
FIELDS = {"silhouette": 0, "position": 1, "depth": 2, "geoNormal": 3, "shNormal": 4, "uv": 5}

_fp = C.c_void_p


class SceneDesc(C.Structure):
    _fields_ = [
        ("width", C.c_int32), ("height", C.c_int32),
        ("num_tris", C.c_int32), ("num_meshes", C.c_int32), ("num_bsdfs", C.c_int32), ("num_emitters", C.c_int32),
        ("num_sec_edges", C.c_int32), ("num_prim_edges", C.c_int32), ("num_texels", C.c_int32),
        ("num_guide_cells", C.c_int32),
        ("tri_info", _fp), ("tri_uv", _fp), ("tri_mesh", _fp), ("mesh_bsdf", _fp), ("mesh_emitter", _fp),
        ("bsdf_rec", _fp), ("texels", _fp), ("emitter_f", _fp), ("emitter_i", _fp),
        ("face_cmf", _fp), ("face_pmf", _fp), ("emitter_cmf", _fp), ("emitter_pmf", _fp),
        ("emitter_sum", C.c_float),
        ("cam", _fp),
        ("sec_edge", _fp), ("sec_cmf", _fp), ("sec_pmf", _fp), ("sec_sum", C.c_float),
        ("prim_edge", _fp), ("prim_cmf", _fp), ("prim_pmf", _fp), ("prim_sum", C.c_float),
        ("guide_reso", C.c_int32 * 3),
        ("guide_cmf", _fp), ("guide_pmf", _fp), ("guide_sum", C.c_float),
        ("env_emitter", C.c_int32), ("env_tex", C.c_int32 * 3), ("env_reso", C.c_int32 * 2),
        ("env_f", _fp), ("env_cmf", _fp), ("env_pmf", _fp), ("env_sum", C.c_float),
        ("material_mask", C.c_uint32),
        ("sec_edge_faces", _fp),
        ("prim_edge_z", _fp),
    ]


class RenderOpts(C.Structure):
    _fields_ = [
        ("integrator", C.c_int32), ("bsdf_samples", C.c_int32), ("light_samples", C.c_int32),
        ("max_depth", C.c_int32), ("hide_emitters", C.c_int32), ("field", C.c_int32),
        ("spp", C.c_int32), ("sppe", C.c_int32), ("sppse", C.c_int32),
        ("spp_begin", C.c_int32), ("spp_end", C.c_int32),
        ("sppe_begin", C.c_int32), ("sppe_end", C.c_int32),
        ("sppse_begin", C.c_int32), ("sppse_end", C.c_int32),
        ("flags", C.c_int32),
        ("rng_offset", C.c_uint64 * 3),
    ]


class Tangents(C.Structure):
    _fields_ = [("d_tri_info", _fp), ("d_texels", _fp), ("d_emitter_rad", _fp), ("d_cam_to_world", _fp),
                ("d_sec_edge", _fp), ("d_prim_edge", _fp), ("d_env_f", _fp)]


class Grads(C.Structure):
    _fields_ = [("g_tri_info", _fp), ("g_texels", _fp), ("g_emitter_rad", _fp), ("g_cam_to_world", _fp),
                ("g_sec_edge", _fp), ("g_prim_edge", _fp), ("g_env_f", _fp)]


TANGENT_FIELDS = ("tri_info", "texels", "emitter_rad", "cam_to_world", "sec_edge", "prim_edge", "env_f")

HIP_SYMBOLS = (
    "psdr_last_error", "psdr_version", "psdr_abi_struct_sizes", "psdr_scene_create", "psdr_scene_destroy", "psdr_scene_set_option", "psdr_scene_set_tables",
    "psdr_bvh_build", "psdr_bvh_stats", "psdr_scene_info", "psdr_trace", "psdr_render_c", "psdr_render_d_fwd", "psdr_render_d_rev",
    "psdr_guide_build", "psdr_get_counters", "psdr_scene_rev_layout", "psdr_scene_seed_info", "psdr_scene_logd_info",
    "psdr_geo_world_vertices_fwd", "psdr_geo_world_vertices_rev", "psdr_geo_tri_rows_fwd", "psdr_geo_tri_rows_rev", "psdr_geo_sec_edges_fwd", "psdr_geo_sec_edges_rev", "psdr_geo_prim_edges_fwd", "psdr_geo_prim_edges_rev",
    "psdr_geo_compact_edges_fwd", "psdr_geo_compact_edges_rev", "psdr_geo_emitter_tables",
    "psdr_geo_world_vertices_jvp", "psdr_geo_tri_rows_jvp", "psdr_geo_sec_edges_jvp", "psdr_geo_prim_edges_jvp", "psdr_geo_compact_edges_jvp",
    "psdr_cube_sample_reuse", "psdr_sample_boundary_segment_direct",
)

HIP_LIB_PATH = os.path.join(PKG_ROOT, "lib", "libpsdr_hip.so")


def use_library(path):
    global HIP_LIB_PATH
    if _hip is not None:
        raise RuntimeError("psdr_cuda._abi.use_library: the library is already loaded (%s)" % HIP_LIB_PATH)
    HIP_LIB_PATH = os.path.abspath(path)


_hip = None


def load_hip():
    global _hip
    if _hip is not None:
        return _hip
    if not os.path.exists(HIP_LIB_PATH):
        raise RuntimeError("libpsdr_hip.so not built (%s): run `python -c 'import __graft_entry__ as g; g.build()'`"
                           % HIP_LIB_PATH)
    lib = C.CDLL(HIP_LIB_PATH)
    lib.psdr_last_error.restype = C.c_char_p
    lib.psdr_version.restype = C.c_char_p
    vp, i32 = C.c_void_p, C.c_int32
    lib.psdr_scene_create.argtypes = [C.POINTER(vp)]
    lib.psdr_scene_destroy.argtypes = [vp]
    lib.psdr_scene_set_option.argtypes = [vp, C.c_char_p, C.c_double]
    lib.psdr_scene_set_tables.argtypes = [vp, C.POINTER(SceneDesc)]
    lib.psdr_bvh_build.argtypes = [vp, vp]
    lib.psdr_trace.argtypes = [vp, i32] + [vp] * 7 + [vp] * 4 + [vp]
    lib.psdr_render_c.argtypes = [vp, C.POINTER(RenderOpts), vp, vp]
    lib.psdr_render_d_fwd.argtypes = [vp, C.POINTER(RenderOpts), i32, C.POINTER(Tangents), vp, vp, vp]
    lib.psdr_render_d_rev.argtypes = [vp, C.POINTER(RenderOpts), vp, vp, C.POINTER(Grads), vp]
    lib.psdr_guide_build.argtypes = [vp, C.POINTER(RenderOpts), C.POINTER(i32), i32, vp, vp]
    lib.psdr_get_counters.argtypes = [vp, C.POINTER(C.c_uint64)]
    lib.psdr_scene_info.argtypes = [vp, C.POINTER(i32)]
    lib.psdr_scene_rev_layout.argtypes = [vp, C.POINTER(i32)]
    lib.psdr_scene_seed_info.argtypes = [vp, C.POINTER(C.c_int64)]
    lib.psdr_scene_logd_info.argtypes = [vp, C.POINTER(C.c_int64)]
    lib.psdr_geo_world_vertices_fwd.argtypes = [i32, vp, vp, vp, vp, vp]
    lib.psdr_geo_world_vertices_rev.argtypes = [i32, vp, vp, vp, vp, vp, vp, vp]
    lib.psdr_geo_tri_rows_fwd.argtypes = [i32, i32, vp, vp, vp, vp, i32, vp]
    lib.psdr_geo_tri_rows_rev.argtypes = [i32, i32, vp, vp, vp, vp, i32, vp, vp, vp]
    lib.psdr_geo_sec_edges_fwd.argtypes = [i32, vp, vp, vp, i32, vp, vp, vp]
    lib.psdr_geo_sec_edges_rev.argtypes = [i32, vp, vp, vp, vp, i32, vp]
    lib.psdr_geo_prim_edges_fwd.argtypes = [i32, vp, vp, vp, vp, i32, vp, vp, vp, vp, vp]
    lib.psdr_geo_prim_edges_rev.argtypes = [i32, vp, vp, vp, vp, vp, vp, vp]
    lib.psdr_geo_compact_edges_fwd.argtypes = [i32, vp, i32, vp, i32, i32, vp, i32, i32, vp, vp, vp, vp, vp, vp, vp, vp]
    lib.psdr_geo_compact_edges_rev.argtypes = [i32, i32, vp, vp, vp, vp]
    lib.psdr_geo_world_vertices_jvp.argtypes = [i32, vp, vp, vp, vp, vp, vp, vp, vp]
    lib.psdr_geo_tri_rows_jvp.argtypes = [i32, i32, vp, vp, vp, vp, i32, vp, vp, vp]
    lib.psdr_geo_sec_edges_jvp.argtypes = [i32, vp, vp, vp, i32, vp, vp]
    lib.psdr_geo_prim_edges_jvp.argtypes = [i32, vp, vp, vp, vp, vp, vp, vp]
    lib.psdr_geo_compact_edges_jvp.argtypes = [i32, i32, vp, vp, vp, vp]
    lib.psdr_geo_emitter_tables.argtypes = [i32, vp, i32, vp, vp, i32, vp, vp, vp, vp, vp, vp, vp, vp, vp, vp]
    lib.psdr_cube_sample_reuse.argtypes = [i32, C.POINTER(i32), vp, vp, C.c_float, i32, i32, vp, vp, vp]
    lib.psdr_sample_boundary_segment_direct.argtypes = [C.POINTER(SceneDesc), i32] + [vp] * 12
    for name in HIP_SYMBOLS:
        if name not in ("psdr_last_error", "psdr_version"):
            getattr(lib, name).restype = C.c_int
    sizes = (C.c_int32 * 4)()
    lib.psdr_abi_struct_sizes(sizes)
    mine = (C.sizeof(SceneDesc), C.sizeof(RenderOpts), C.sizeof(Tangents), C.sizeof(Grads))
    if tuple(sizes) != mine:
        raise RuntimeError("psdr_cuda/_abi.py is out of sync with include/psdr_hip.h: %s vs %s" % (tuple(sizes), mine))
    _hip = lib
    return lib


def check(lib, rc):
    if rc != 0:
        msg = lib.psdr_last_error()
        raise RuntimeError(msg.decode() if msg else "psdr_hip call failed (rc=%d)" % rc)


def scene_stats(handle):
    lib = load_hip()
    out = (C.c_int32 * 8)()
    check(lib, lib.psdr_scene_info(handle, out))
    return {"n_tiny": out[0], "n_blas": out[1], "n_inline": out[2], "leaf_tris": out[3], "device_built": out[4], "n_slab": out[5], "occ_rows": out[6], "occ_max_rows": out[7]}


REV_LAUNCH_KINDS = {-1: "none", 0: "fused", 1: "split", 2: "split_wavefront", 3: "kept_records", 4: "probe"}


def rev_layout(handle):
    lib = load_hip()
    out = (C.c_int32 * 16)()
    check(lib, lib.psdr_scene_rev_layout(handle, out))
    return {"tex_n": out[0], "rad_n": out[1], "env_n": out[2], "hot_rows": out[3], "rep": out[4], "priv_rows": out[5], "priv_regs": out[6],
            "pend_rows": out[7], "launch": REV_LAUNCH_KINDS[out[8]], "pe_reps": out[9], "hot_identity": out[10], "deep_rec": out[11],
            "priv_slot": (out[12], out[13]), "tree_hot_rows": out[14], "pe_sorted": out[15]}


def seed_cache_info(handle):
    lib = load_hip()
    out = (C.c_int64 * 4)()
    check(lib, lib.psdr_scene_seed_info(handle, out))
    return {"slots": int(out[0]), "bytes": int(out[1]), "fills": int(out[2]), "launches": int(out[3])}


def logd_info(handle):
    lib = load_hip()
    out = (C.c_int64 * 4)()
    check(lib, lib.psdr_scene_logd_info(handle, out))
    return {"launches": int(out[0]), "lean": int(out[1]), "lean_seeded": int(out[2]), "lean_lds_bytes": int(out[3])}


def make_opts(integrator=INTEGRATOR_DIRECT, bsdf_samples=1, light_samples=1, max_depth=1, hide_emitters=False,
              field=0, spp=1, sppe=0, sppse=0, spp_range=None, sppe_range=None, sppse_range=None,
              rng_offset=(0, 0, 0), flags=0):
    o = RenderOpts()
    o.flags = flags
    o.integrator, o.bsdf_samples, o.light_samples = integrator, bsdf_samples, light_samples
    o.max_depth, o.hide_emitters, o.field = max_depth, int(bool(hide_emitters)), field
    o.spp, o.sppe, o.sppse = spp, sppe, sppse
    o.spp_begin, o.spp_end = spp_range if spp_range is not None else (0, spp)
    o.sppe_begin, o.sppe_end = sppe_range if sppe_range is not None else (0, sppe)
    o.sppse_begin, o.sppse_end = sppse_range if sppse_range is not None else (0, sppse)
    for i in range(3):
        o.rng_offset[i] = int(rng_offset[i])
    return o


def draws_per_slot(opts):
    if opts.integrator == INTEGRATOR_DIRECT:
        li = 3 * opts.bsdf_samples + 2 * opts.light_samples
    elif opts.integrator == INTEGRATOR_PATH:
        li = 5 * opts.max_depth
    else:
        li = 0
    se = 3
    if opts.integrator == INTEGRATOR_PATH and (opts.flags & FLAG_PATH_SEDGES) and opts.max_depth >= 2:
        se = 11 * opts.max_depth - 9
    return (2 + li, 1 + 2 * li, se)
```

Before: 20680 Mpath-samples/s.

## Stage per-primitive vertex rows in LDS for tiny-scene camera kernels

Adds a new translation unit with specialised camera kernels for render C and the lean logd render D. At block start they pack each tiny primitive's triangle data, UVs, mesh, BSDF record and emitter radiance into 52-word rows in LDS, plus a triangle-to-row map. Hits are then resolved straight against these rows through a raw closest_hit mode, which avoids scattered global-table lookups per bounce. The cost is extra LDS per block, which may lower occupancy, and a larger code path that falls back when the rows do not fit.

```diff
diff --git a/__graft_entry__.py b/__graft_entry__.py
--- a/__graft_entry__.py
+++ b/__graft_entry__.py
@@ -40,6 +40,10 @@
         o = os.path.join(obj_dir, "logd_lean.o")
         objs.append(o)
         unit_cmds[o] = ["hipcc"] + HIPCC_FLAGS + ["-c", os.path.join(csrc, "psdr_logd_lean.hip"), "-o", o]
+        jobs.append(subprocess.Popen(unit_cmds[o]))
+        o = os.path.join(obj_dir, "vertex_rows.o")
+        objs.append(o)
+        unit_cmds[o] = ["hipcc"] + HIPCC_FLAGS + ["-c", os.path.join(csrc, "psdr_vertex_rows.hip"), "-o", o]
         jobs.append(subprocess.Popen(unit_cmds[o]))
         o = os.path.join(obj_dir, "host.o")
         objs.append(o)
@@ -113,7 +117,7 @@
     srcs = [os.path.join(csrc, f) for f in os.listdir(csrc)] + [os.path.join(ROOT, "include", "psdr_hip.h")]
     obj_dir = os.path.join(PKG, "lib", "obj")
     defect_lib = os.path.join(ROOT, "tests", "poison", "libpsdr_hip_defect.so")
-    objs = [os.path.join(obj_dir, "%s%d.o" % (unit, v)) for v in VARIANTS for unit in ("variant", "path_sedge")] + [os.path.join(obj_dir, "logd_lean.o"), os.path.join(obj_dir, "host.o"), os.path.join(obj_dir, "tables.o")]
+    objs = [os.path.join(obj_dir, "%s%d.o" % (unit, v)) for v in VARIANTS for unit in ("variant", "path_sedge")] + [os.path.join(obj_dir, "logd_lean.o"), os.path.join(obj_dir, "vertex_rows.o"), os.path.join(obj_dir, "host.o"), os.path.join(obj_dir, "tables.o")]
     if not all(os.path.exists(o) for o in objs):
         return None
     if object_job is not None and object_job.wait() != 0:
diff --git a/include/psdr_hip.h b/include/psdr_hip.h
--- a/include/psdr_hip.h
+++ b/include/psdr_hip.h
@@ -208,6 +208,10 @@
 
 int psdr_scene_logd_info(psdr_scene_t h, int64_t out[4]);
 
+int psdr_scene_rows_info(psdr_scene_t h, int64_t out[4]);
+
+int psdr_scene_vertex_rows(psdr_scene_t h, uint32_t *out_words, int32_t capacity_words, int32_t info[4], void *stream);
+
 int psdr_get_counters(psdr_scene_t h, uint64_t out[4]);
 
 #ifdef __cplusplus
diff --git a/psdr-cuda_amd/csrc/psdr_device.h b/psdr-cuda_amd/csrc/psdr_device.h
--- a/psdr-cuda_amd/csrc/psdr_device.h
+++ b/psdr-cuda_amd/csrc/psdr_device.h
@@ -434,8 +434,8 @@
     return x;
 #endif
 }
-template <bool IGN = false, int FOREST = -1, bool MASKED = false>
-PSDR_HD Hit closest_hit(const SceneView &sc, TraversalStack &st, const Vec3f &o, const Vec3f &d, float tmax, int ig0 = -1, int ig1 = -1, int pre_slot = 0, uint32_t rows = 0xffffffffu) {
+template <bool IGN = false, int FOREST = -1, bool MASKED = false, bool RAW = false>
+PSDR_HD Hit closest_hit(const SceneView &sc, TraversalStack &st, const Vec3f &o, const Vec3f &d, float tmax, int ig0 = -1, int ig1 = -1, int pre_slot = 0, uint32_t rows = 0xffffffffu, int *raw = nullptr) {
     Hit best; best.tri = -1; best.u = best.v = -1.f;
     best.t = (tmax > 0.f && tmax < INFINITY) ? __int_as_float_hd(__float_as_int_hd(tmax) + 1) : tmax;
     const Vec3f inv{1.f / d.x, 1.f / d.y, 1.f / d.z};
@@ -474,6 +474,7 @@
 #pragma unroll PSDR_TINY_UNROLL
         for (int i = aa_cnt != 0 ? kAaSlots : 0; i < sc.n_tiny; ++i)
             if (!MASKED || ((rows >> i) & 1u) != 0u) tiny_prim_test<IGN>(prim_rows[i * 4], prim_rows[i * 4 + 1], prim_rows[i * 4 + 2], prim_rows[i * 4 + 3], i, o, d, best, best_i, ig0, ig1);
+        if constexpr (RAW) { static_assert(FOREST == 2, "unresolved hits: scenes without a tree"); *raw = best_i; return best; }
         resolve_tiny_hit(sc, best, best_i);
         if (FOREST == 3) {
             const Hit ph = st.pre[pre_slot];
@@ -831,6 +832,7 @@
     const MatCache<M> *mc = nullptr;
     PSDR_HD Bsdf(const SceneView &sc, int id) : rec(sc.d.bsdf_rec + (size_t) (id < 0 ? 0 : id) * PSDR_BSDF_STRIDE) {}
     template <class TVT> PSDR_HD Bsdf(const SceneView &sc, const TVT &, int id) : rec(Tab<TVT::flags>::bsdf_rec(sc, id)) {}
+    PSDR_HD explicit Bsdf(const int32_t *record) : rec(record) {}
     template <class TVT> PSDR_HD MatCache<M> fetch(const SceneView &sc, const TVT &tv, const Its<G> &its) const {
         MatCache<M> c;
         c.refl = tex3(sc, tv, PSDR_SLOT_REFLECTANCE, its);
diff --git a/psdr-cuda_amd/csrc/psdr_hip.hip b/psdr-cuda_amd/csrc/psdr_hip.hip
--- a/psdr-cuda_amd/csrc/psdr_hip.hip
+++ b/psdr-cuda_amd/csrc/psdr_hip.hip
@@ -499,6 +499,26 @@
     return off + stack_bytes;
 }
 int lds_bytes(const LaunchCtx &cx, const psdr_scene_s *h) { return cx.off_stack + stack_entries_of(h) * kBlock * 4; }
+bool plan_vertex_rows(const psdr_scene_s *h, LaunchCtx &cx, RowPlan &rp) {
+    SceneView &sc = cx.sc;
+    if (h->opt.vertex_rows == 0 || !tiny_tables_ok(h) || h->has_rough || h->desc.env_emitter >= 0 || sc.lt_trimesh < 0 || sc.n_tiny <= 0) return false;
+    const psdr_scene_desc &d = h->desc;
+    int off = 0;
+    auto take = [&](int words) { const int o = off; off += (words * 4 + 15) / 16 * 16; return o; };
+    rp.n_rows = 2 * sc.n_tiny;
+    rp.off_rows = take(rp.n_rows * kRowWords);
+    rp.off_map = take(d.num_tris);
+    sc.n_lnodes = sc.n_lbtris = sc.n_ltri = 0; sc.off_lnodes = sc.off_lbtris = sc.off_ltri = sc.off_lprim = 0;
+    sc.lt_trimesh = sc.lt_meshbsdf = sc.lt_meshemitter = sc.lt_bsdf = sc.lt_uv = -1;
+    sc.lt_emf = take(d.num_emitters * PSDR_EMITTER_F_STRIDE); sc.lt_emi = take(d.num_emitters * PSDR_EMITTER_I_STRIDE);
+    sc.lt_fcmf = take(sc.lt_nfaces); sc.lt_fpmf = take(sc.lt_nfaces);
+    if (sc.lt_ecmf >= 0) { sc.lt_ecmf = take(d.num_emitters); sc.lt_epmf = take(d.num_emitters); }
+    if (sc.lt_tex >= 0) sc.lt_tex = take(d.num_texels * (1 + kLdsTexelTangents));
+    if (sc.lt_occ >= 0) sc.lt_occ = take(d.num_tris * d.num_tris);
+    sc.lt_end = off;
+    cx.off_stack = off;
+    return true;
+}
 
 void fill_top(const psdr_scene_s *h, SceneView &sc) {
     sc.n_tiny = h->n_tiny; sc.aa_cnt = h->n_tiny > 0 ? h->aa_cnt : 0;
@@ -937,6 +957,7 @@
     else if (n == "logd") h->opt.logd = iv;
     else if (n == "seed_cache") h->opt.seed_cache = iv;
     else if (n == "logd_park") h->opt.logd_park = iv;
+    else if (n == "vertex_rows") h->opt.vertex_rows = iv;
     else if (n == "seed_cache_log2") h->opt.seed_cache_log2 = std::max(0, std::min(40, iv));
     else if (n == "keep_records") h->opt.keep_records = iv;
     else if (n == "rev_sorted") h->opt.rev_sorted = iv;
@@ -1394,6 +1415,17 @@
     out[0] = h->logd_launches; out[1] = h->logd_lean_launches; out[2] = h->logd_lean_seeded; out[3] = (int64_t) h->logd_lean_lds + h->logd_lean_park;
     return 0;
 }
+int psdr_scene_rows_info(psdr_scene_t h, int64_t out[4]) {
+    if (!h || !out) return fail("psdr_scene_rows_info: null argument");
+    out[0] = h->rows_launches_c; out[1] = h->rows_launches_d; out[2] = h->rows_lds; out[3] = h->rows_bytes;
+    return 0;
+}
+int psdr_scene_vertex_rows(psdr_scene_t h, uint32_t *out_words, int32_t capacity_words, int32_t info[4], void *stream) {
+    if (!h || !info) return fail("psdr_scene_vertex_rows: null argument");
+    if (!h->have_tables) return fail("Scene not loaded yet!");
+    if (!h->have_bvh) return fail("Input scene must be configured!");
+    return vertex_rows_dump_8(h, out_words, capacity_words, info, (hipStream_t) stream);
+}
 int psdr_scene_seed_info(psdr_scene_t h, int64_t out[4]) {
     if (!h || !out) return fail("psdr_scene_seed_info: null argument");
     out[0] = h->seed_valid ? h->seed_key[0] * h->seed_key[3] : 0; out[1] = (int64_t) (h->seed_cap * sizeof(ulonglong2)); out[2] = h->seed_fills; out[3] = h->seed_launches;
diff --git a/psdr-cuda_amd/csrc/psdr_host.h b/psdr-cuda_amd/csrc/psdr_host.h
--- a/psdr-cuda_amd/csrc/psdr_host.h
+++ b/psdr-cuda_amd/csrc/psdr_host.h
@@ -21,6 +21,14 @@
     int32_t off_pathrec;
     int32_t off_sink;
     int32_t off_park;
+};
+
+constexpr int kRowWords = 52, kRowBytes = kRowWords * 4;
+constexpr int kRowUv = 24, kRowTri = 30, kRowMesh = 31, kRowK = 32, kRowBsdfId = 38, kRowEmitter = 39, kRowBsdf = 40, kRowRadiance = 44, kRowEf3 = 47, kRowEf4 = 48;
+struct RowPlan {
+    int32_t off_rows;
+    int32_t off_map;
+    int32_t n_rows;
 };
 
 static_assert(offsetof(LaunchCtx, sc) == 0, "closest_hit reads SceneView::tiny through the kernel-argument segment pointer: LaunchCtx (SceneView first) must be the first kernel argument");
@@ -139,6 +147,7 @@
     int seed_cache = 1;
     int seed_cache_log2 = 25;
     int logd_park = 1;
+    int vertex_rows = 1;
     int bvh_maxleaf = 4;
     float bvh_tcost = 2.0f;
 };
@@ -229,6 +238,7 @@
     hipEvent_t seed_event = nullptr;
     long long seed_fills = 0, seed_launches = 0;
     long long logd_launches = 0, logd_lean_launches = 0, logd_lean_seeded = 0;
+    long long rows_launches_c = 0, rows_launches_d = 0; int rows_lds = 0, rows_bytes = 0;
     int logd_lean_lds = 0, logd_lean_park = 0;
     void *d_ws = nullptr;
     size_t ws_bytes = 0;
@@ -288,6 +298,10 @@
 const PathSedgeOps *path_sedge_ops_8();
 const PathSedgeOps *path_sedge_ops_10();
 int logd_lean_launch_8(psdr_scene_s *h, const psdr_render_opts *o, const LaunchCtx &cx, const psdr::TangentView<1, psdr::kSceneTiny> &tv, float *img, float *dimg, hipStream_t s, bool *ran);
+bool plan_vertex_rows(const psdr_scene_s *h, LaunchCtx &cx, RowPlan &rp);
+int vertex_rows_launch_c_8(psdr_scene_s *h, const psdr_render_opts *o, const LaunchCtx &cx, float *img, hipStream_t s, const ulonglong2 *seed, bool *ran);
+int vertex_rows_launch_d_8(psdr_scene_s *h, const psdr_render_opts *o, const LaunchCtx &cx, const psdr::TangentView<1, psdr::kSceneTiny> &tv, float *img, float *dimg, hipStream_t s, bool *ran, bool *no_lean);
+int vertex_rows_dump_8(psdr_scene_s *h, uint32_t *out_words, int capacity_words, int32_t info[4], hipStream_t s);
 const VariantOps *variant_ops_0();
 const VariantOps *variant_ops_1();
 const VariantOps *variant_ops_2();
diff --git a/psdr-cuda_amd/csrc/psdr_kernels.h b/psdr-cuda_amd/csrc/psdr_kernels.h
--- a/psdr-cuda_amd/csrc/psdr_kernels.h
+++ b/psdr-cuda_amd/csrc/psdr_kernels.h
@@ -1585,7 +1585,11 @@
             hipLaunchKernelGGL(k_logd_check<K>, dim3((unsigned) ((h->desc.num_texels + kBlock - 1) / kBlock)), dim3(kBlock), 0, s, h->desc.texels, tvk, h->desc.num_texels, h->d_counters, bad);
             hipLaunchKernelGGL(k_logd_gate, dim3(1), dim3(64), 0, s, h->d_counters, bad);
             bool lean = false;
-            if constexpr (K == 1 && FL == kSceneTiny) { if (int rc = logd_lean_launch_8(h, o, cx, tv, img, dimg, s, &lean)) return rc; }
+            if constexpr (K == 1 && FL == kSceneTiny) {
+                bool no_lean = false;
+                if (int rc = vertex_rows_launch_d_8(h, o, cx, tv, img, dimg, s, &lean, &no_lean)) return rc;
+                if (!lean && !no_lean) { if (int rc = logd_lean_launch_8(h, o, cx, tv, img, dimg, s, &lean)) return rc; }
+            }
             if (!lean)
                 hipLaunchKernelGGL(HIP_KERNEL_NAME(k_camera_logd<K, FL, ((FL & kSceneTiny) != 0)>), dim3(launch_blocks(h, n, camera_blocks_per_cu(h, n))), dim3(kBlock), lds_bytes(cx, h), s, cx, tv,
                                    o->spp, o->spp_begin, SlotDiv(nsp), n, 1.f / (float) o->spp, img, dimg, WH * 3, h->d_counters, own);
@@ -1601,6 +1605,11 @@
     if constexpr (seeded_render_c<G, R, FL>()) {
         if (o->integrator == PSDR_INTEGRATOR_PATH) {
             if (const ulonglong2 *seed = seed_table(h, o, WH, nsp, n, s)) {
+                if constexpr (FL == kSceneTiny) {
+                    bool rows = false;
+                    if (int rc = vertex_rows_launch_c_8(h, o, cx, img, s, seed, &rows)) return rc;
+                    if (rows) { HIP_TRY(hipGetLastError()); h->seed_launches++; return 0; }
+                }
                 hipLaunchKernelGGL(HIP_KERNEL_NAME(k_camera_seeded<G, R, PSDR_INTEGRATOR_PATH, FL, true>), dim3(launch_blocks(h, n, camera_blocks_per_cu(h, n))), dim3(kBlock), lds_bytes(cx, h), s, cx, tv,
                                    o->spp, o->spp_begin, SlotDiv(nsp), n, 1.f / (float) o->spp, img, dimg, WH * 3, h->d_counters, own, seed);
                 HIP_TRY(hipGetLastError());
diff --git a/psdr-cuda_amd/csrc/psdr_vertex_rows.h b/psdr-cuda_amd/csrc/psdr_vertex_rows.h
--- /dev/null
+++ b/psdr-cuda_amd/csrc/psdr_vertex_rows.h
@@ -0,0 +1,426 @@
+#pragma once
+#include "psdr_host.h"
+#include "psdr_logd_lean.h"
+
+namespace psdr {
+
+struct RowIts : Its<float> { int rowb; };
+PSDR_HD const float *row_f(int rowb) { return PSDR_LDS_TABLE(float, rowb); }
+PSDR_HD const int32_t *row_i(int rowb) { return PSDR_LDS_TABLE(int32_t, rowb); }
+
+__device__ __forceinline__ void stage_vertex_rows(const SceneView &sc, const RowPlan &rp) {
+#if defined(__HIP_DEVICE_COMPILE__)
+    typedef __attribute__((address_space(4))) const char kernarg_char;
+    kernarg_char *args = (kernarg_char *) __builtin_amdgcn_kernarg_segment_ptr();
+    const int32_t *meta_tab = (const int32_t *) (const char *) (args + offsetof(SceneView, tiny_meta));
+    const float4 *prim_tab = (const float4 *) (const char *) (args + offsetof(SceneView, tiny));
+    uint32_t *rows = reinterpret_cast<uint32_t *>(psdr_dyn_lds + rp.off_rows);
+    int32_t *map = reinterpret_cast<int32_t *>(psdr_dyn_lds + rp.off_map);
+    const int t = threadIdx.x, T = sc.d.num_tris;
+    for (int i = t; i < T; i += kBlock) map[i] = rp.off_rows;
+    int32_t tri = -1;
+    if (t < rp.n_rows) {
+        const int prim = t >> 1;
+        const int32_t meta[4] = {meta_tab[prim * 4], meta_tab[prim * 4 + 1], meta_tab[prim * 4 + 2], meta_tab[prim * 4 + 3]};
+        const float4 Sm = prim_tab[prim * 4 + 2];
+        const float S[4] = {Sm.x, Sm.y, Sm.z, Sm.w};
+        float k[6];
+        const bool slab = sc.aa_cnt != 0 && prim < kAaSlots;
+        tiny_hit_row(meta, t & 1, tri, k, slab ? S : nullptr);
+        const int ax = slab ? prim / kAaPerAxis : 0, cnt = (sc.aa_cnt >> (8 * ax)) & 255;
+        if ((slab && prim - ax * kAaPerAxis >= cnt) || tri < 0 || tri >= T) tri = -1;
+        uint32_t *r = rows + t * kRowWords;
+        r[kRowTri] = (uint32_t) tri;
+#pragma unroll
+        for (int j = 0; j < 6; ++j) r[kRowK + j] = tri >= 0 ? __float_as_uint(k[j]) : 0u;
+    }
+    __syncthreads();
+    if (t < rp.n_rows && tri >= 0 && (t & 1) == 0) map[tri] = rp.off_rows + t * kRowBytes;
+    __syncthreads();
+    if (t < rp.n_rows && tri >= 0 && (t & 1) == 1 && rows[(t - 1) * kRowWords + kRowTri] != (uint32_t) tri) map[tri] = rp.off_rows + t * kRowBytes;
+    const uint32_t *tri_info = reinterpret_cast<const uint32_t *>(sc.d.tri_info), *tri_uv = reinterpret_cast<const uint32_t *>(sc.d.tri_uv);
+    for (int i = t; i < rp.n_rows * 32; i += kBlock) {
+        const int row = i >> 5, w = i & 31;
+        const int32_t tr = (int32_t) rows[row * kRowWords + kRowTri];
+        if (w >= kRowTri) continue;
+        uint32_t v = 0u;
+        if (tr >= 0) v = w < kRowUv ? tri_info[(size_t) tr * PSDR_TRI_STRIDE + w] : (tri_uv != nullptr ? tri_uv[(size_t) tr * PSDR_TRIUV_STRIDE + (w - kRowUv)] : 0u);
+        rows[row * kRowWords + w] = v;
+    }
+    if (t < rp.n_rows) {
+        uint32_t *r = rows + t * kRowWords;
+        int32_t tm = 0, bsdf_id = 0, em = 0;
+        uint32_t rec[4] = {0u, 0u, 0u, 0u}, ef[5] = {0u, 0u, 0u, 0u, 0u};
+        if (tri >= 0) {
+            tm = sc.d.tri_mesh[tri];
+            const int mesh = tm & ~PSDR_TRI_FACE_NORMALS;
+            bsdf_id = sc.d.mesh_bsdf[mesh]; em = sc.d.mesh_emitter[mesh];
+            const uint32_t *br = reinterpret_cast<const uint32_t *>(sc.d.bsdf_rec) + (size_t) (bsdf_id < 0 ? 0 : bsdf_id) * PSDR_BSDF_STRIDE;
+#pragma unroll
+            for (int j = 0; j < 4; ++j) rec[j] = br[j];
+            if (em >= 0) {
+                const uint32_t *e = reinterpret_cast<const uint32_t *>(sc.d.emitter_f) + (size_t) em * PSDR_EMITTER_F_STRIDE;
+#pragma unroll
+                for (int j = 0; j < 5; ++j) ef[j] = e[j];
+            }
+        }
+        r[kRowMesh] = (uint32_t) tm; r[kRowBsdfId] = (uint32_t) bsdf_id; r[kRowEmitter] = (uint32_t) em;
+#pragma unroll
+        for (int j = 0; j < 4; ++j) r[kRowBsdf + j] = rec[j];
+#pragma unroll
+        for (int j = 0; j < 5; ++j) r[kRowRadiance + j] = ef[j];
+        r[49] = r[50] = r[51] = 0u;
+    }
+#else
+    (void) sc; (void) rp;
+#endif
+}
+__device__ __forceinline__ void setup_lds_rows(const LaunchCtx &cx, const RowPlan &rp, TraversalStack &st) {
+#if defined(__HIP_DEVICE_COMPILE__)
+    const SceneView &sc = cx.sc;
+    stage_vertex_rows(sc, rp);
+    auto stage = [&](int off, const void *table, int words) {
+        if (off < 0 || table == nullptr) return;
+        const uint32_t *g = static_cast<const uint32_t *>(table);
+        uint32_t *l = reinterpret_cast<uint32_t *>(psdr_dyn_lds + off);
+#pragma unroll 1
+        for (int i = threadIdx.x; i < words; i += kBlock) l[i] = g[i];
+    };
+    stage(sc.lt_emf, sc.d.emitter_f, sc.d.num_emitters * PSDR_EMITTER_F_STRIDE);
+    stage(sc.lt_emi, sc.d.emitter_i, sc.d.num_emitters * PSDR_EMITTER_I_STRIDE);
+    stage(sc.lt_ecmf, sc.d.emitter_cmf, sc.d.num_emitters);
+    stage(sc.lt_epmf, sc.d.emitter_pmf, sc.d.num_emitters);
+    stage(sc.lt_fcmf, sc.d.face_cmf, sc.lt_nfaces);
+    stage(sc.lt_fpmf, sc.d.face_pmf, sc.lt_nfaces);
+    stage(sc.lt_tex, sc.d.texels, sc.d.num_texels);
+    stage(sc.lt_occ, sc.occ, sc.d.num_tris * sc.d.num_tris);
+    st.base = reinterpret_cast<int32_t *>(psdr_dyn_lds + cx.off_stack) + threadIdx.x;
+    __syncthreads();
+#else
+    (void) cx; (void) rp; (void) st;
+#endif
+}
+
+template <class TVT> __device__ __forceinline__ void setup_lds_rows(const LaunchCtx &cx, const RowPlan &rp, TraversalStack &st, const TVT &tv) {
+    setup_lds_rows(cx, rp, st);
+#if defined(__HIP_DEVICE_COMPILE__)
+    constexpr int K = TVT::k;
+    static_assert(K >= 1 && K <= 3, "plan_lds reserves three tangent texel pools");
+    if (cx.sc.lt_tex >= 0) {
+        float *l = reinterpret_cast<float *>(psdr_dyn_lds + cx.sc.lt_tex);
+        const int nt = cx.sc.d.num_texels;
+        for (int k = 0; k < K; ++k) {
+            const float *g = tv.t[k].d_texels;
+            for (int i = threadIdx.x; i < nt; i += kBlock) l[(k + 1) * nt + i] = g ? g[i] : 0.f;
+        }
+        __syncthreads();
+    }
+#else
+    (void) tv;
+#endif
+}
+
+PSDR_HD TriRow<float> row_tri(const float4 (&r)[6]) {
+    TriRow<float> t;
+    t.p0 = {r[0].x, r[0].y, r[0].z}; t.e1 = {r[0].w, r[1].x, r[1].y}; t.e2 = {r[1].z, r[1].w, r[2].x};
+    t.n0 = {r[2].y, r[2].z, r[2].w}; t.n1 = {r[3].x, r[3].y, r[3].z}; t.n2 = {r[3].w, r[4].x, r[4].y};
+    t.fn = {r[4].z, r[4].w, r[5].x}; t.area = r[5].y;
+    return t;
+}
+
+template <bool MASKED = false>
+PSDR_HD RowIts intersect_rows(const SceneView &sc, const RowPlan &rp, TraversalStack &st, const RayT<float> &ray, bool active, uint32_t &nrays, uint32_t occ = 0xffffffffu) {
+    RowIts its;
+    its.valid = false; its.tri = its.mesh = -1; its.J = 1.f; its.t = INFINITY; its.rowb = rp.off_rows;
+    if (!active) return its;
+    nrays++;
+    int packed = kNoPrim;
+    const Hit h = closest_hit<false, 2, MASKED, true>(sc, st, ray.o, ray.d, INFINITY, -1, -1, 0, MASKED ? wave_or_hd(occ) : 0xffffffffu, &packed);
+    if (packed == kNoPrim) return its;
+    const bool plane = (uint32_t) packed < (uint32_t) kNoPrim;
+    const float rho = plane ? 1.f : __int_as_float_hd(packed);
+    const int best_i = plane ? packed : (packed & 15);
+    const int half = h.u * rho + h.v > 0.f ? 1 : 0;
+    its.rowb = rp.off_rows + (best_i * 2 + half) * kRowBytes;
+    const float4 *q = PSDR_LDS_TABLE(float4, its.rowb);
+    float4 r[6];
+#pragma unroll
+    for (int i = 0; i < 6; ++i) r[i] = q[i];
+    const float4 ua = q[6], ub = q[7], ka = q[8], kb = q[9];
+    float k[6];
+    k[0] = ka.x; k[1] = ka.y; k[2] = ka.z; k[3] = ka.w; k[4] = kb.x; k[5] = kb.y;
+    const float u = h.u, v = h.v;
+    const float hu = k[0] + (k[1] * u + k[2] * v);
+    const float hv = k[3] + (k[4] * u + k[5] * v);
+    its.valid = true; its.tri = __float_as_int_hd(ub.z); its.hu = hu; its.hv = hv;
+    const int tm = __float_as_int_hd(ub.w);
+    const TriRow<float> T = row_tri(r);
+    its.n = T.fn;
+    const float bu = hu, bv = hv;
+    its.p = bary_point(T.p0, T.e1, T.e2, bu, bv);
+    Vec3f dir = its.p - ray.o;
+    its.t = norm(dir);
+    dir = dir / its.t;
+    Vec3f sh_n = (tm & PSDR_TRI_FACE_NORMALS) ? its.n : normalize(bary_point(T.n0, T.n1 - T.n0, T.n2 - T.n0, bu, bv));
+    its.sh = Frame<float>(sh_n);
+    its.wi = its.sh.to_local(-dir);
+    if (sc.d.tri_uv) {
+        const float qq[6] = {ua.x, ua.y, ua.z, ua.w, ub.x, ub.y};
+        its.uvx = (qq[2] - qq[0]) * bu + ((qq[4] - qq[0]) * bv + qq[0]);
+        its.uvy = (qq[3] - qq[1]) * bu + ((qq[5] - qq[1]) * bv + qq[1]);
+    } else { its.uvx = 0.f; its.uvy = 0.f; }
+    return its;
+}
+
+PSDR_HD int emitter_of(const RowIts &its) { return its.valid ? row_i(its.rowb)[kRowEmitter] : -1; }
+PSDR_HD Vec3f Le_rows(const RowIts &its, bool active) {
+    const int e = active ? emitter_of(its) : -1;
+    if (e < 0) return zero3<float>();
+    if (!(its.wi.z > 0.f)) return zero3<float>();
+    const float *f = row_f(its.rowb) + kRowRadiance;
+    return {f[0], f[1], f[2]};
+}
+PSDR_HD float emitter_position_pdf_rows(const RowIts &its) {
+    const int e = emitter_of(its);
+    if (e < 0) return 0.f;
+    const float *f = row_f(its.rowb);
+    return f[kRowEf3] * f[kRowEf4];
+}
+template <class TVT>
+PSDR_HD PosSample<float> sample_emitter_position_rows(const SceneView &sc, const RowPlan &rp, const TVT &, float s0, float s1) {
+    static_assert(!TVT::has_env, "rows: no environment map");
+    PosSample<float> ps;
+    int e = 0; float epdf = 1.f;
+    if (sc.d.num_emitters > 1) e = sample_reuse(Tab<TVT::flags>::emitter_cmf(sc), Tab<TVT::flags>::emitter_pmf(sc), sc.d.emitter_sum, sc.d.num_emitters, s1, epdf);
+    const float *ef = Tab<TVT::flags>::emitter_f(sc, e);
+    const int32_t *ei = Tab<TVT::flags>::emitter_i(sc, e);
+    float fp;
+    const int f = sample_reuse(Tab<TVT::flags>::face_cmf(sc) + ei[3], Tab<TVT::flags>::face_pmf(sc) + ei[3], ef[5], ei[2], s0, fp);
+    const float t = sqrtf(fmaxf(1.f - s0, 0.f));
+    const float4 *q = PSDR_LDS_TABLE(float4, PSDR_LDS_TABLE(int32_t, rp.off_map)[ei[1] + f]);
+    float4 r[6];
+#pragma unroll
+    for (int i = 0; i < 6; ++i) r[i] = q[i];
+    const TriRow<float> T = row_tri(r);
+    ps.J = 1.f;
+    ps.p = bary_point(T.p0, T.e1, T.e2, float(1.f - t), float(t * s1));
+    ps.n = T.fn;
+    ps.pdf = ef[4] * epdf;
+    ps.valid = true;
+    ps.tri = ei[1] + f;
+    return ps;
+}
+
+template <class TVT>
+PSDR_HD Vec3f path_vertex_rows(const SceneView &sc, const RowPlan &rp, const TVT &tv, TraversalStack &st, Rng &rng, const RowIts &its, bool active, uint32_t &nrays,
+                               RowIts &next_its, Vec3f &next_f, bool &next_valid) {
+    static_assert(TVT::tiny && !TVT::has_env && !TVT::has_rough && TVT::k == 0, "rows serve the plain diffuse flag set of scenes without a tree");
+    Vec3f result = zero3<float>();
+    int bsdf_id = active ? row_i(its.rowb)[kRowBsdfId] : 0;
+    if (bsdf_id < 0) { active = false; bsdf_id = 0; }
+    const Bsdf<float, float> bsdf(row_i(its.rowb) + kRowBsdf);
+    const float s[3] = {rng.next(), rng.next(), rng.next()};
+    const float s0 = rng.next(), s1 = rng.next();
+    if (!active) return result;
+    {
+        const PosSample<float> ps = sample_emitter_position_rows(sc, rp, tv, s0, s1);
+        Vec3f wo = ps.p - its.p;
+        const float d2 = dot(wo, wo), dist = safe_sqrt(d2);
+        wo = wo / dist;
+        const RayT<float> ray1{its.p, wo};
+        const Vec3f wl = its.sh.to_local(wo);
+        const bool lit = PSDR_SKIP_UNLIT ? (wl.z > 0.f && its.wi.z > 0.f) : true;
+        const RowIts its1 = PSDR_OCC_ROWS ? intersect_rows<true>(sc, rp, st, ray1, ps.valid && lit, nrays, occ_rows(sc, its.tri, ps.tri))
+                                          : intersect_rows<false>(sc, rp, st, ray1, ps.valid && lit, nrays);
+        if (its1.valid && its1.t > dist - kShadowEpsilon && emitter_of(its1) >= 0) {
+            const float Gv = abs_(dot(its1.n, -wo)) / d2;
+            const Vec3f bsdf_val = bsdf.eval(sc, tv, its, wl, true) * to_m<float>(Gv * ps.J / ps.pdf);
+            float pdf1 = bsdf.pdf(sc, tv, its, wl, true);
+            pdf1 = pdf1 * Gv;
+            const float w = mis_weight(float(ps.pdf), pdf1);
+            result = result + Le_rows(its1, true) * bsdf_val * w;
+        }
+    }
+    {
+        Vec3f wo_s; float pdf_s;
+        bool a1 = bsdf.sample(sc, tv, its, s, active, wo_s, pdf_s);
+        const Vec3f dir1{fmaf(its.sh.n.x, wo_s.z, fmaf(wo_s.x, its.sh.s.x, __fmul_rn(wo_s.y, its.sh.t.x))),
+                         fmaf(its.sh.n.y, wo_s.z, fmaf(wo_s.x, its.sh.s.y, __fmul_rn(wo_s.y, its.sh.t.y))),
+                         fmaf(its.sh.n.z, wo_s.z, fmaf(wo_s.y, its.sh.t.z, __fmul_rn(wo_s.x, its.sh.s.z)))};
+        const RayT<float> ray1{its.p, dir1};
+        const RowIts its1 = intersect_rows<false>(sc, rp, st, ray1, a1, nrays);
+        const bool a_hit = a1 && its1.valid;
+        a1 = a_hit && emitter_of(its1) >= 0;
+        Vec3f bsdf_val = zero3<float>(); float pdf0(0.f);
+        if (a_hit) {
+            bsdf_val = bsdf.eval(sc, tv, its, wo_s, true);
+            const float Gv = abs_(dot(its1.n, -ray1.d)) / sqr(its1.t);
+            pdf0 = pdf_s * Gv;
+            bsdf_val = bsdf_val / pdf_s;
+        }
+        if (a1) {
+            const float w = mis_weight(pdf0, float(emitter_position_pdf_rows(its1)));
+            result = result + Le_rows(its1, true) * bsdf_val * w;
+        }
+        next_its = its1; next_f = bsdf_val; next_valid = a_hit;
+    }
+    return result;
+}
+
+template <class TVT>
+PSDR_HD Vec3f li_path_rows(const SceneView &sc, const RowPlan &rp, const TVT &tv, TraversalStack &st, const LiParams &lp, Rng &rng, const RayT<float> &ray, uint32_t &nrays) {
+    RowIts its = intersect_rows<false>(sc, rp, st, ray, true, nrays);
+    bool active = its.valid;
+    Vec3f result = lp.hide_emitters ? zero3<float>() : Le_rows(its, active);
+    Vec3f beta(1.f);
+    for (int depth = 0; depth < lp.max_depth; ++depth) {
+        RowIts nits; Vec3f nf; bool nvalid = false;
+        const Vec3f c = path_vertex_rows(sc, rp, tv, st, rng, its, active, nrays, nits, nf, nvalid);
+        if (active) {
+            result = result + beta * c;
+            active = nvalid;
+            if (active) {
+                beta = beta * nf;
+                its = nits;
+                if (!(beta.x != 0.f || beta.y != 0.f || beta.z != 0.f)) active = false;
+            }
+        }
+    }
+    return result;
+}
+
+template <int K, class TVT>
+PSDR_HD void albedo_logd_rows(const SceneView &sc, const TVT &tv, const RowIts &its, float (&g)[K][3]) {
+    const int bsdf_id = row_i(its.rowb)[kRowBsdfId];
+#pragma unroll
+    for (int k = 0; k < K; ++k) g[k][0] = g[k][1] = g[k][2] = 0.f;
+    if (bsdf_id < 0) return;
+    const Bsdf<float, Dual<K>> bsdf(row_i(its.rowb) + kRowBsdf);
+    const Vec3<Dual<K>> rho = bsdf.tex3(sc, tv, PSDR_SLOT_REFLECTANCE, its);
+    const float ix = rho.x.v != 0.f ? 1.f / rho.x.v : 0.f, iy = rho.y.v != 0.f ? 1.f / rho.y.v : 0.f, iz = rho.z.v != 0.f ? 1.f / rho.z.v : 0.f;
+#pragma unroll
+    for (int k = 0; k < K; ++k) { g[k][0] = rho.x.d[k] * ix; g[k][1] = rho.y.d[k] * iy; g[k][2] = rho.z.d[k] * iz; }
+}
+
+template <int K, class TVT>
+__device__ __forceinline__ Vec3<Dual<K>> li_path_logd_lean_rows(const SceneView &sc, const RowPlan &rp, const TVT &tv, TraversalStack &st, const LiParams &lp, Rng &rng, const RayT<float> &ray,
+                                                              bool active0, uint32_t &nrays, const Park &pk) {
+    using L = ParkLayout<K>;
+    using TV0 = TangentView<0, TVT::flags>;
+    static_assert(TVT::tiny && !TVT::has_env && !TVT::has_rough, "rows serve the plain diffuse flag set of scenes without a tree");
+    const TV0 tv0{};
+    RowIts its = intersect_rows<false>(sc, rp, st, ray, active0, nrays);
+    bool active = active0 && its.valid;
+    Vec3f result = lp.hide_emitters ? Vec3f(0.f) : Le_rows(its, active);
+    float rd[K][3], s[K][3];
+#pragma unroll
+    for (int k = 0; k < K; ++k) { rd[k][0] = rd[k][1] = rd[k][2] = 0.f; s[k][0] = s[k][1] = s[k][2] = 0.f; }
+    Vec3f beta(1.f);
+    for (int depth = 0; depth < lp.max_depth; ++depth) {
+        if (active) {
+            float g[K][3];
+            albedo_logd_rows<K>(sc, tv, its, g);
+#pragma unroll
+            for (int k = 0; k < K; ++k) { s[k][0] += g[k][0]; s[k][1] += g[k][1]; s[k][2] += g[k][2]; }
+        }
+        int bsdf_id = active ? row_i(its.rowb)[kRowBsdfId] : 0;
+        bool act = active;
+        if (bsdf_id < 0) { act = false; bsdf_id = 0; }
+        const Bsdf<float, float> bsdf(row_i(its.rowb) + kRowBsdf);
+        const float sb0 = rng.next(), sb1 = rng.next(), sb2 = rng.next();
+        const float s0 = rng.next(), s1 = rng.next();
+        pk.put3(L::result, result); pk.put3(L::beta, beta);
+#pragma unroll
+        for (int k = 0; k < K; ++k) {
+            pk.put(L::rd + 3 * k, rd[k][0]); pk.put(L::rd + 3 * k + 1, rd[k][1]); pk.put(L::rd + 3 * k + 2, rd[k][2]);
+            pk.put(L::s + 3 * k, s[k][0]); pk.put(L::s + 3 * k + 1, s[k][1]); pk.put(L::s + 3 * k + 2, s[k][2]);
+        }
+        pk.put64(L::rng, rng.state); pk.put64(L::rng + 2, rng.inc);
+        pk.put(L::vtx, sb1); pk.put(L::vtx + 1, sb2);
+        Park::fence();
+        Vec3f c(0.f);
+        if (act) {
+            const PosSample<float> ps = sample_emitter_position_rows(sc, rp, tv0, s0, s1);
+            Vec3f wo = ps.p - its.p;
+            const float d2 = dot(wo, wo), dist = safe_sqrt(d2);
+            wo = wo / dist;
+            const RayT<float> ray1{its.p, wo};
+            const Vec3f wl = its.sh.to_local(wo);
+            const bool lit = PSDR_SKIP_UNLIT ? (wl.z > 0.f && its.wi.z > 0.f) : true;
+            const RowIts its1 = PSDR_OCC_ROWS ? intersect_rows<true>(sc, rp, st, ray1, ps.valid && lit, nrays, occ_rows(sc, its.tri, ps.tri))
+                                              : intersect_rows<false>(sc, rp, st, ray1, ps.valid && lit, nrays);
+            if (its1.valid && its1.t > dist - kShadowEpsilon && emitter_of(its1) >= 0) {
+                const float Gv = abs_(dot(its1.n, -wo)) / d2;
+                const Vec3f bsdf_val = bsdf.eval(sc, tv0, its, wl, true) * to_m<float>(Gv * ps.J / ps.pdf);
+                float pdf1 = bsdf.pdf(sc, tv0, its, wl, true);
+                pdf1 = pdf1 * Gv;
+                const float w = mis_weight(float(ps.pdf), pdf1);
+                c = c + Le_rows(its1, true) * bsdf_val * w;
+            }
+        }
+        Park::fence();
+        const float sb[3] = {sb0, pk.get(L::vtx), pk.get(L::vtx + 1)};
+        Park::fence();
+        pk.put3(L::vtx, c);
+        Park::fence();
+        RowIts nits; Vec3f nf(0.f); bool nvalid = false;
+        Vec3f lb(0.f); float wb = 0.f; bool a1b = false;
+        if (act) {
+            Vec3f wo_s; float pdf_s;
+            bool a1 = bsdf.sample(sc, tv0, its, sb, true, wo_s, pdf_s);
+            Vec3f shn = its.sh.n;
+            asm volatile("" : "+v"(shn.x), "+v"(shn.y), "+v"(shn.z));
+            const Frame<float> fr(shn);
+            const Vec3f dir1 = fr.s * wo_s.x + fr.t * wo_s.y + shn * wo_s.z;
+            const RayT<float> ray1{its.p, dir1};
+            const RowIts its1 = intersect_rows<false>(sc, rp, st, ray1, a1, nrays);
+            const bool a_hit = a1 && its1.valid;
+            a1 = a_hit && emitter_of(its1) >= 0;
+            Vec3f bsdf_val(0.f); float pdf0(0.f);
+            if (a_hit) {
+                bsdf_val = bsdf.eval(sc, tv0, its, wo_s, true);
+                const float Gv = abs_(dot(its1.n, -ray1.d)) / sqr(its1.t);
+                pdf0 = pdf_s * Gv;
+                bsdf_val = bsdf_val / pdf_s;
+            }
+            if (a1) {
+                wb = mis_weight(pdf0, float(emitter_position_pdf_rows(its1)));
+                lb = Le_rows(its1, true) * bsdf_val;
+            }
+            a1b = a1;
+            nits = its1; nf = bsdf_val; nvalid = a_hit;
+        }
+        Park::fence();
+        c = pk.get3(L::vtx);
+        result = pk.get3(L::result); beta = pk.get3(L::beta);
+#pragma unroll
+        for (int k = 0; k < K; ++k) {
+            rd[k][0] = pk.get(L::rd + 3 * k); rd[k][1] = pk.get(L::rd + 3 * k + 1); rd[k][2] = pk.get(L::rd + 3 * k + 2);
+            s[k][0] = pk.get(L::s + 3 * k); s[k][1] = pk.get(L::s + 3 * k + 1); s[k][2] = pk.get(L::s + 3 * k + 2);
+        }
+        rng.state = pk.get64(L::rng); rng.inc = pk.get64(L::rng + 2);
+        Park::fence();
+        if (a1b) c = c + lb * wb;
+        if (active) {
+            const Vec3f bc = beta * c;
+            result = result + bc;
+#pragma unroll
+            for (int k = 0; k < K; ++k) {
+                rd[k][0] = fmaf(bc.x, s[k][0], rd[k][0]); rd[k][1] = fmaf(bc.y, s[k][1], rd[k][1]); rd[k][2] = fmaf(bc.z, s[k][2], rd[k][2]);
+            }
+            active = nvalid;
+            if (active) {
+                beta = beta * nf;
+                if (!(beta.x != 0.f || beta.y != 0.f || beta.z != 0.f)) active = false;
+            }
+        }
+        its = nits;
+    }
+    Vec3<Dual<K>> out;
+    out.x.v = result.x; out.y.v = result.y; out.z.v = result.z;
+#pragma unroll
+    for (int k = 0; k < K; ++k) { out.x.d[k] = rd[k][0]; out.y.d[k] = rd[k][1]; out.z.d[k] = rd[k][2]; }
+    return out;
+}
+
+}
diff --git a/psdr-cuda_amd/csrc/psdr_vertex_rows.hip b/psdr-cuda_amd/csrc/psdr_vertex_rows.hip
--- /dev/null
+++ b/psdr-cuda_amd/csrc/psdr_vertex_rows.hip
@@ -0,0 +1,189 @@
+#define PSDR_WIDE_TREE 0
+#define PSDR_LEAF_PAIR 0
+#include "psdr_kernels.h"
+#include "psdr_vertex_rows.h"
+
+namespace {
+
+constexpr int kRowsFlags = kSceneTiny;
+
+__global__ __launch_bounds__(kBlock, (camera_waves<float, float, PSDR_INTEGRATOR_PATH, kRowsFlags, true>())) void k_camera_rows(LaunchCtx cx, RowPlan rp, SlotDiv nsp, long long n, float inv_spp,
+                                                                                                                                 float *__restrict__ img, unsigned long long *counters, int own,
+                                                                                                                                 const ulonglong2 *__restrict__ seed) {
+    TraversalStack st; setup_lds_rows(cx, rp, st);
+    const TangentView<0, kRowsFlags> tv{};
+    uint32_t nrays = 0;
+    const long long nceil = (n + kBlock - 1) / kBlock * kBlock;
+    for (long long j = (long long) blockIdx.x * kBlock + threadIdx.x; j < nceil; j += (long long) gridDim.x * kBlock) {
+        const bool in = j < n;
+        const ulonglong2 sd = in ? seed[j] : ulonglong2{0ull, 0ull};
+        int pixel = 0x7fffffff, s_in = 0;
+        if (in) slot_to_pixel(j, nsp, pixel, s_in);
+        float v[3] = {0.f, 0.f, 0.f};
+        if (in) {
+            Rng rng = seeded_rng(sd, cx.jump);
+            const float j0 = rng.next(), j1 = rng.next();
+            const int W = cx.sc.d.width;
+            const int px = pixel % W, py = pixel / W;
+            const float sx = ((float) px + j0) / (float) W, sy = ((float) py + j1) / (float) cx.sc.d.height;
+            const RayT<float> ray = primary_ray<float>(cx.sc, tv, sx, sy);
+            const Vec3f r = zero_nonfinite(li_path_rows(cx.sc, rp, tv, st, cx.lp, rng, ray, nrays));
+            v[0] = r.x * inv_spp; v[1] = r.y * inv_spp; v[2] = r.z * inv_spp;
+        }
+        const bool head = wave_segmented_sum<3>(pixel, v);
+        if (head && in) {
+            float *p = img + (size_t) pixel * 3;
+            if (own) { p[0] = v[0]; p[1] = v[1]; p[2] = v[2]; }
+            else {
+                if (v[0] != 0.f) atomicAdd(p, v[0]);
+                if (v[1] != 0.f) atomicAdd(p + 1, v[1]);
+                if (v[2] != 0.f) atomicAdd(p + 2, v[2]);
+            }
+        }
+    }
+    count_rays(counters, nrays);
+}
+
+template <int K>
+__global__ __launch_bounds__(kBlock, PSDR_LOGD_WAVES_K1) void k_camera_logd_rows(LaunchCtx cx, RowPlan rp, TV<Dual<K>, kRowsFlags> tv, SlotDiv nsp, long long n, float inv_spp,
+                                                                                  float *__restrict__ img, float *__restrict__ dimg, long long plane, unsigned long long *counters, int own,
+                                                                                  const ulonglong2 *__restrict__ seed) {
+    constexpr int NV = 3 * (1 + K);
+    if (counters[kLogdGateWord] != 1ull) return;
+    TraversalStack st; setup_lds_rows(cx, rp, st, tv);
+    Park pk{nullptr};
+#if defined(__HIP_DEVICE_COMPILE__)
+    pk.base = reinterpret_cast<float *>(psdr_dyn_lds + cx.off_park) + threadIdx.x;
+#endif
+    uint32_t nrays = 0;
+    const long long nceil = (n + kBlock - 1) / kBlock * kBlock;
+    for (long long jb = (long long) blockIdx.x * kBlock; jb < nceil; jb += (long long) gridDim.x * kBlock) {
+        const long long j = jb + threadIdx.x;
+        const bool in = j < n;
+        int pixel = 0x7fffffff, s_in = 0;
+        if (in) slot_to_pixel(j, nsp, pixel, s_in);
+        Rng rng;
+        const ulonglong2 sd = in ? seed[j] : ulonglong2{0ull, 0ull};
+        rng.init_seeded(sd.x, sd.y, cx.jump);
+        const float j0 = rng.next(), j1 = rng.next();
+        const int W = cx.sc.d.width;
+        const float sx = ((float) (pixel % W) + j0) / (float) W, sy = ((float) (pixel / W) + j1) / (float) cx.sc.d.height;
+        const TangentView<0, kRowsFlags> tv0{};
+        const RayT<float> ray = primary_ray<float>(cx.sc, tv0, sx, sy);
+        const Vec3<Dual<K>> r = zero_nonfinite(li_path_logd_lean_rows<K>(cx.sc, rp, tv, st, cx.lp, rng, ray, in, nrays, pk));
+        float v[NV];
+        v[0] = in ? r.x.v * inv_spp : 0.f; v[1] = in ? r.y.v * inv_spp : 0.f; v[2] = in ? r.z.v * inv_spp : 0.f;
+#pragma unroll
+        for (int k = 0; k < K; ++k) { v[3 + 3 * k] = in ? r.x.d[k] * inv_spp : 0.f; v[4 + 3 * k] = in ? r.y.d[k] * inv_spp : 0.f; v[5 + 3 * k] = in ? r.z.d[k] * inv_spp : 0.f; }
+        const bool head = wave_segmented_sum<NV>(pixel, v);
+        if (head && in) {
+            float *p = img + (size_t) pixel * 3;
+            if (own) {
+                p[0] = v[0]; p[1] = v[1]; p[2] = v[2];
+#pragma unroll
+                for (int k = 0; k < K; ++k) { float *q = dimg + (size_t) k * plane + (size_t) pixel * 3; q[0] = v[3 + 3 * k]; q[1] = v[4 + 3 * k]; q[2] = v[5 + 3 * k]; }
+            } else {
+                if (v[0] != 0.f) atomicAdd(p, v[0]);
+                if (v[1] != 0.f) atomicAdd(p + 1, v[1]);
+                if (v[2] != 0.f) atomicAdd(p + 2, v[2]);
+#pragma unroll
+                for (int k = 0; k < K; ++k) {
+                    float *q = dimg + (size_t) k * plane + (size_t) pixel * 3;
+                    if (v[3 + 3 * k] != 0.f) atomicAdd(q, v[3 + 3 * k]);
+                    if (v[4 + 3 * k] != 0.f) atomicAdd(q + 1, v[4 + 3 * k]);
+                    if (v[5 + 3 * k] != 0.f) atomicAdd(q + 2, v[5 + 3 * k]);
+                }
+            }
+        }
+    }
+    count_rays(counters, nrays);
+}
+
+__global__ __launch_bounds__(kBlock) void k_rows_dump(LaunchCtx cx, RowPlan rp, uint32_t *__restrict__ out, int words) {
+    TraversalStack st; setup_lds_rows(cx, rp, st);
+#if defined(__HIP_DEVICE_COMPILE__)
+    const int nr = rp.n_rows * kRowWords, nt = cx.sc.d.num_tris;
+    const uint32_t *rows = reinterpret_cast<const uint32_t *>(psdr_dyn_lds + rp.off_rows);
+    const int32_t *map = reinterpret_cast<const int32_t *>(psdr_dyn_lds + rp.off_map);
+    for (int i = threadIdx.x; i < nr && i < words; i += kBlock) out[i] = rows[i];
+    for (int i = threadIdx.x; i < nt && nr + i < words; i += kBlock) out[nr + i] = (uint32_t) ((map[i] - rp.off_rows) / kRowBytes);
+    typedef __attribute__((address_space(4))) const char kernarg_char;
+    kernarg_char *args = (kernarg_char *) __builtin_amdgcn_kernarg_segment_ptr();
+    const uint32_t *meta = (const uint32_t *) (const char *) (args + offsetof(SceneView, tiny_meta));
+    const uint32_t *prim = (const uint32_t *) (const char *) (args + offsetof(SceneView, tiny));
+    const int np = rp.n_rows / 2, base = nr + nt;
+    for (int i = threadIdx.x; i < np * 4 && base + np * 8 < words; i += kBlock) {
+        out[base + i] = meta[i];
+        out[base + np * 4 + i] = prim[(i >> 2) * 16 + 8 + (i & 3)];
+    }
+    if (threadIdx.x == 0 && base + np * 8 < words) out[base + np * 8] = (uint32_t) cx.sc.aa_cnt;
+#else
+    (void) out; (void) words;
+#endif
+}
+
+}
+
+namespace psdr_host {
+static bool rows_fit(const psdr_scene_s *h, int bytes, int waves) {
+    constexpr int kCuLds = 160 * 1024;
+    return bytes <= (h->opt.lds_budget > 0 ? std::min(h->opt.lds_budget, kCuLds / waves) : kCuLds / waves);
+}
+int vertex_rows_launch_c_8(psdr_scene_s *h, const psdr_render_opts *o, const LaunchCtx &cx0, float *img, hipStream_t s, const ulonglong2 *seed, bool *ran) {
+    *ran = false;
+    LaunchCtx cx = cx0;
+    RowPlan rp;
+    if (seed == nullptr || !plan_vertex_rows(h, cx, rp)) return 0;
+    const int lds = (lds_bytes(cx, h) + 15) / 16 * 16;
+    if (!rows_fit(h, lds, camera_waves<float, float, PSDR_INTEGRATOR_PATH, kRowsFlags, true>())) return 0;
+    const long long WH = (long long) h->desc.width * h->desc.height;
+    const int nsp = o->spp_end - o->spp_begin;
+    const long long n = WH * nsp;
+    const int own = (h->opt.own_pixels != 0 && nsp <= 64 && 64 % nsp == 0) ? 1 : 0;
+    hipLaunchKernelGGL(k_camera_rows, dim3(launch_blocks(h, n, camera_blocks_per_cu(h, n))), dim3(kBlock), lds, s, cx, rp, SlotDiv(nsp), n, 1.f / (float) o->spp, img, h->d_counters, own, seed);
+    h->rows_launches_c++;
+    h->rows_lds = lds; h->rows_bytes = rp.n_rows * kRowBytes;
+    *ran = true;
+    return 0;
+}
+int vertex_rows_launch_d_8(psdr_scene_s *h, const psdr_render_opts *o, const LaunchCtx &cx0, const psdr::TangentView<1, psdr::kSceneTiny> &tv, float *img, float *dimg, hipStream_t s, bool *ran, bool *no_lean) {
+    *ran = false; *no_lean = false;
+    if (h->opt.logd_park == 0) return 0;
+    LaunchCtx cx = cx0;
+    RowPlan rp;
+    if (!plan_vertex_rows(h, cx, rp)) return 0;
+    constexpr int kCuLds = 160 * 1024, park = ParkLayout<1>::cols * kBlock * 4;
+    const int lds = (lds_bytes(cx, h) + 15) / 16 * 16;
+    if (lds + park > kCuLds / PSDR_LOGD_WAVES_K1) return 0;
+    if (!rows_fit(h, lds + park, PSDR_LOGD_WAVES_K1)) { *no_lean = true; return 0; }
+    const long long WH = (long long) h->desc.width * h->desc.height;
+    const int nsp = o->spp_end - o->spp_begin;
+    const long long n = WH * nsp;
+    const ulonglong2 *seed = seed_table(h, o, WH, nsp, n, s);
+    if (seed == nullptr) return 0;
+    cx.off_park = lds;
+    const int own = (h->opt.own_pixels != 0 && nsp <= 64 && 64 % nsp == 0) ? 1 : 0;
+    hipLaunchKernelGGL(HIP_KERNEL_NAME(k_camera_logd_rows<1>), dim3(launch_blocks(h, n, camera_blocks_per_cu(h, n))), dim3(kBlock), lds + park, s, cx, rp, tv, SlotDiv(nsp), n, 1.f / (float) o->spp, img, dimg,
+                       WH * 3, h->d_counters, own, seed);
+    h->logd_lean_launches++; h->logd_lean_seeded++; h->seed_launches++;
+    h->logd_lean_lds = lds; h->logd_lean_park = park;
+    h->rows_launches_d++;
+    h->rows_lds = lds + park; h->rows_bytes = rp.n_rows * kRowBytes;
+    *ran = true;
+    return 0;
+}
+int vertex_rows_dump_8(psdr_scene_s *h, uint32_t *out_words, int capacity_words, int32_t info[4], hipStream_t s) {
+    psdr_render_opts o{};
+    o.integrator = PSDR_INTEGRATOR_PATH; o.max_depth = 1; o.spp = o.spp_end = 1;
+    LaunchCtx cx;
+    if (int rc = make_ctx(h, &o, 0, cx)) return rc;
+    RowPlan rp;
+    if (!plan_vertex_rows(h, cx, rp)) return fail("psdr_scene_vertex_rows: the scene has no vertex rows (option vertex_rows 0, a tree, or another flag set than plain diffuse)");
+    info[0] = rp.n_rows; info[1] = kRowWords; info[2] = h->desc.num_tris; info[3] = (lds_bytes(cx, h) + 15) / 16 * 16;
+    if (out_words == nullptr) return 0;
+    if (capacity_words < rp.n_rows * kRowWords + h->desc.num_tris + rp.n_rows * 4 + 1) return fail("psdr_scene_vertex_rows: the buffer is too small");
+    hipLaunchKernelGGL(k_rows_dump, dim3(1), dim3(kBlock), info[3], s, cx, rp, out_words, capacity_words);
+    HIP_TRY(hipGetLastError());
+    return 0;
+}
+}
diff --git a/psdr-cuda_amd/psdr_cuda/_abi.py b/psdr-cuda_amd/psdr_cuda/_abi.py
--- a/psdr-cuda_amd/psdr_cuda/_abi.py
+++ b/psdr-cuda_amd/psdr_cuda/_abi.py
@@ -78,7 +78,7 @@
 HIP_SYMBOLS = (
     "psdr_last_error", "psdr_version", "psdr_abi_struct_sizes", "psdr_scene_create", "psdr_scene_destroy", "psdr_scene_set_option", "psdr_scene_set_tables",
     "psdr_bvh_build", "psdr_bvh_stats", "psdr_scene_info", "psdr_trace", "psdr_render_c", "psdr_render_d_fwd", "psdr_render_d_rev",
-    "psdr_guide_build", "psdr_get_counters", "psdr_scene_rev_layout", "psdr_scene_seed_info", "psdr_scene_logd_info",
+    "psdr_guide_build", "psdr_get_counters", "psdr_scene_rev_layout", "psdr_scene_seed_info", "psdr_scene_logd_info", "psdr_scene_rows_info", "psdr_scene_vertex_rows",
     "psdr_geo_world_vertices_fwd", "psdr_geo_world_vertices_rev", "psdr_geo_tri_rows_fwd", "psdr_geo_tri_rows_rev", "psdr_geo_sec_edges_fwd", "psdr_geo_sec_edges_rev", "psdr_geo_prim_edges_fwd", "psdr_geo_prim_edges_rev",
     "psdr_geo_compact_edges_fwd", "psdr_geo_compact_edges_rev", "psdr_geo_emitter_tables",
     "psdr_geo_world_vertices_jvp", "psdr_geo_tri_rows_jvp", "psdr_geo_sec_edges_jvp", "psdr_geo_prim_edges_jvp", "psdr_geo_compact_edges_jvp",
@@ -124,6 +124,8 @@
     lib.psdr_scene_rev_layout.argtypes = [vp, C.POINTER(i32)]
     lib.psdr_scene_seed_info.argtypes = [vp, C.POINTER(C.c_int64)]
     lib.psdr_scene_logd_info.argtypes = [vp, C.POINTER(C.c_int64)]
+    lib.psdr_scene_rows_info.argtypes = [vp, C.POINTER(C.c_int64)]
+    lib.psdr_scene_vertex_rows.argtypes = [vp, vp, i32, C.POINTER(i32), vp]
     lib.psdr_geo_world_vertices_fwd.argtypes = [i32, vp, vp, vp, vp, vp]
     lib.psdr_geo_world_vertices_rev.argtypes = [i32, vp, vp, vp, vp, vp, vp, vp]
     lib.psdr_geo_tri_rows_fwd.argtypes = [i32, i32, vp, vp, vp, vp, i32, vp]
@@ -193,6 +195,28 @@
     return {"launches": int(out[0]), "lean": int(out[1]), "lean_seeded": int(out[2]), "lean_lds_bytes": int(out[3])}
 
 
+def rows_info(handle):
+    lib = load_hip()
+    out = (C.c_int64 * 4)()
+    check(lib, lib.psdr_scene_rows_info(handle, out))
+    return {"render_c": int(out[0]), "logd": int(out[1]), "lds_bytes": int(out[2]), "row_bytes": int(out[3])}
+
+
+def vertex_rows(handle):
+    import torch
+    lib = load_hip()
+    info = (C.c_int32 * 4)()
+    check(lib, lib.psdr_scene_vertex_rows(handle, None, 0, info, None))
+    n_rows, words, n_tris = info[0], info[1], info[2]
+    buf = torch.zeros(n_rows * words + n_tris + n_rows * 4 + 1, dtype=torch.int32, device="cuda")
+    check(lib, lib.psdr_scene_vertex_rows(handle, buf.data_ptr(), buf.numel(), info, None))
+    torch.cuda.synchronize()
+    buf = buf.cpu()
+    a, b, c = n_rows * words, n_rows * words + n_tris, n_rows * words + n_tris + n_rows * 2
+    return {"rows": buf[:a].reshape(n_rows, words), "tri_to_row": buf[a:b], "codes": buf[b:c].reshape(-1, 4), "slab_map": buf[c:c + n_rows * 2].reshape(-1, 4),
+            "aa_cnt": int(buf[-1]), "lds_bytes": int(info[3])}
+
+
 def make_opts(integrator=INTEGRATOR_DIRECT, bsdf_samples=1, light_samples=1, max_depth=1, hide_emitters=False,
               field=0, spp=1, sppe=0, sppse=0, spp_range=None, sppe_range=None, sppse_range=None,
               rng_offset=(0, 0, 0), flags=0):
```

New measurement: 21680 Mpath-samples/s (median of 5 runs). +4.8%, better.
